# yangt1013/SPEINet

Measured on AMD Instinct MI355X. Metric: deblurred 720p frames/sec, higher is better.
Workload: dtype f16 (correlation top2)

## Files before the change

include/speinet_hip.h:

```cpp
#ifndef SPEINET_HIP_H
#define SPEINET_HIP_H

#include <stdint.h>

#ifdef __cplusplus
extern "C" {
#endif

typedef void* spei_stream_t;

#define SPEI_ACT_NONE 0
#define SPEI_ACT_RELU 1
#define SPEI_ACT_GELU 2

#define SPEI_F32 0
#define SPEI_BF16 1
#define SPEI_F16 2

#define SPEI_CONV 0
#define SPEI_CONV_TRANSPOSED 1

int spei_version(void);
const char* spei_last_error(void);
const char* spei_arch(void);

int spei_any_nonzero(const float* x, int64_t n, int32_t* flag, spei_stream_t stream);

int spei_rl_prior(const float* img, float* out, float* scratch, int C, int H, int W, int iters, float lam,
                  spei_stream_t stream);

int spei_conv5_in(const float* img_chw, const float* w, const float* bias, float* out_hwc, int H, int W,
                  int Cout, spei_stream_t stream);

int spei_conv5_out(const float* in_hwc, int ldi, const float* w, const float* bias, float* out_chw, int H,
                   int W, int Cin, spei_stream_t stream);

int spei_igemm_f32(const float* a0, int lda0, int k0, const float* a1, int lda1, int k1, const float* w,
                   const float* bias, float* out, int ldo, const float* residual, int ldr,
                   const float* rowscale, int Hin, int Win, int Hout, int Wout, int N, int ksize, int stride,
                   int pad, int mode, int act, spei_stream_t stream);

int spei_igemm_f32_batched(const float* a0, int lda0, int k0, const float* a1, int lda1, int k1, const float* w,
                           const float* bias, float* out, int ldo, const float* residual, int ldr,
                           const float* rowscale, int Hin, int Win, int Hout, int Wout, int N, int ksize, int stride,
                           int pad, int mode, int act, int batch, spei_stream_t stream);

int spei_conv_slab16(int fmt, const void* a0, int lda0, int k0, const void* a1, int lda1, int k1, int a_fmt,
                     const void* wfrag_hi, const void* wfrag_lo, const float* bias, void* out, int ldo, int out_fmt,
                     const float* residual, int ldr, const float* rowscale, int Hin, int Win, int Hout, int Wout,
                     int N, int ksize, int stride, int pad, int act, int ln_input, spei_stream_t stream);

int spei_conv_slab16_batched(int fmt, const void* a0, int k0, int a_fmt, const void* wfrag, const void* wfrag_lo, const float* bias,
                             void* out, int out_fmt, const float* residual, int batch, int Hin, int Win, int Hout, int Wout, int N,
                             int ksize, int stride, int pad, int act, spei_stream_t stream);

int spei_conv32_ws16(int fmt, const void* a, int a_fmt, const void* wfrag, const float* bias, void* out, int out_fmt, int batch,
                     int H, int W, int act, spei_stream_t stream);

int spei_conv64_ws16(int fmt, const void* a, int a_fmt, const void* wfrag, const float* bias, void* out, int out_fmt, int batch,
                     int H, int W, int act, spei_stream_t stream);

int spei_mlp_fused16(int fmt, const float* x, float* out, const void* w1_frag, const float* b1, const void* w2_frag,
                     const float* b2, int64_t M, spei_stream_t stream);

int spei_convt2_slab16(int fmt, const void* a0, int lda0, int k0, int a_fmt, const void* wfrag00, const void* wfrag01,
                       const void* wfrag10, const void* wfrag11, const float* bias, void* out, int ldo, int out_fmt,
                       int Hin, int Win, int N, int act, spei_stream_t stream);

int spei_convt2_slab16x3(const float* a0, int lda0, int k0, const void* const* whi4, const void* const* wlo4, const float* bias,
                         float* out, int ldo, int Hin, int Win, int N, int act, spei_stream_t stream);

int spei_conv3x3_256_pipe16(int fmt, const float* x, const void* w_frag, const float* bias, const float* residual, float* out,
                            int batch, int H, int W, spei_stream_t stream);

int spei_conv5_out_slab16(int fmt, const void* in, int ldi, int in_fmt, const void* wfrag, const float* bias32, float* out_chw,
                          int H, int W, spei_stream_t stream);

int spei_attn_fused16(int fmt, const float* x, float* out, const void* yhat, const void* wq_frag, const float* bq,
                      const void* wkv_frag, const float* bkv, const void* wproj_frag, const float* bproj,
                      const float* relbias, int H, int W, int shift, spei_stream_t stream);

int spei_attn_win4_16(int fmt, const float* x, float* out, const void* yhat, const void* wq_frag, const float* bq,
                      const void* wkv_frag, const float* bkv, const void* wproj_frag, const float* bproj,
                      const float* relbias, int batch, int H, int W, int shift, spei_stream_t stream);

int64_t spei_frame_metrics_ws_doubles(int H, int W, int border);
int spei_frame_metrics(const unsigned char* out_hwc, const unsigned char* gt_hwc, int H, int W, int border, double* ws, double* result,
                       spei_stream_t stream);

int64_t spei_gate_ws_floats(int H, int W, int C);
int spei_resblock_gates(const void* x1, int x1_fmt, int H, int W, int C, const float* se_w1, const float* se_b1,
                        const float* se_w2, const float* se_b2, const float* cw_w, const float* cw_bn,
                        const float* hc_w, const float* hc_bn, float* s, float* g1, float* g2, float* ws,
                        spei_stream_t stream);
int spei_resblock_apply(const float* x, const void* x1, int x1_fmt, const float* s, const float* g1, const float* g2,
                        const float* extra, float* out, int ldo, int H, int W, int C, spei_stream_t stream);

int spei_resblock_gates_batched(const void* x1, int x1_fmt, int batch, int H, int W, int C, const float* se_w1, const float* se_b1,
                                const float* se_w2, const float* se_b2, const float* cw_w, const float* cw_bn, const float* hc_w,
                                const float* hc_bn, float* s, float* g1, float* g2, float* ws, spei_stream_t stream);
int spei_resblock_apply_batched(const float* x, const void* x1, int x1_fmt, const float* s, const float* g1, const float* g2, float* out,
                                int batch, int H, int W, int C, spei_stream_t stream);

int spei_layernorm256(const float* x, void* y, int out_fmt, const float* gamma, const float* beta, int64_t M,
                      spei_stream_t stream);

int spei_window_attention(const void* q, const void* kv, int io_fmt, const float* relbias, void* out, int H, int W,
                          int shift, spei_stream_t stream);
int spei_window_attention_batched(const void* q, const void* kv, int io_fmt, const float* relbias, void* out, int H, int W,
                                  int shift, int batch, spei_stream_t stream);

int spei_patch_invnorm(const float* f, int ldf, float* inv, int H, int W, int C, spei_stream_t stream);

int64_t spei_corr_ws_floats(int64_t n_lr);
int spei_corr_argmax(const float* lr, int ldl, const float* ref, int ldr, const float* inv_lr,
                     const float* inv_ref, int Hl, int Wl, int Hr, int Wr, int C, float* S, int32_t* arg,
                     float* ws, spei_stream_t stream);

int spei_split16(int fmt, const float* x, int ld, void* hi, void* lo, int64_t M, int C, spei_stream_t stream);
int spei_corr_argmax_bf16(const void* lr_hi, const void* lr_lo, const void* ref_hi, const void* ref_lo,
                          const float* inv_lr, const float* inv_ref, int Hl, int Wl, int Hr, int Wr, int C, float* S,
                          int32_t* arg, float* ws, spei_stream_t stream);

int spei_corr_slab16(int fmt, const void* lr_hi, const void* lr_lo, const void* ref_hi, const void* ref_lo,
                     const float* inv_lr, const float* inv_ref, int Hl, int Wl, int Hr, int Wr, int C, float* S,
                     int32_t* arg, float* ws, spei_stream_t stream);

int spei_corr_slab_top2_16(int fmt, const void* lr16, const void* ref16, const float* inv_lr, const float* inv_ref,
                           int Hl, int Wl, int Hr, int Wr, int C, float* S, int32_t* arg, float* S2, int32_t* arg2,
                           float* ws, spei_stream_t stream);
int64_t spei_corr_diag_ws_floats(int Hl, int Wl, int Hr, int Wr);
int spei_corr_diag_top2_16(int fmt, const void* lr16, const void* ref16, const float* inv_ref, int Hl, int Wl, int Hr, int Wr,
                           int C, float* S, int32_t* arg, float* S2, int32_t* arg2, float* ws, spei_stream_t stream);
int spei_corr_rescore(const float* lr, int ldl, const float* ref, int ldr, const float* inv_lr, const float* inv_ref,
                      int Hl, int Wl, int Hr, int Wr, int C, float* S, int32_t* arg, const float* S2, const int32_t* arg2,
                      spei_stream_t stream);

int spei_gather_fold(const float* ref, int ldr, const int32_t* arg, float* out, int ldo, int H3, int W3,
                     int Hr3, int Wr3, int C, int s, spei_stream_t stream);

int spei_rot90(const float* in, int ldi, float* out, int H, int W, int C, spei_stream_t stream);

int spei_upsample_bicubic(const float* in, int ldi, float* out, int ldo, int H, int W, int C, int s, int act,
                          spei_stream_t stream);

int spei_add(const float* a, const float* b, float* out, int64_t n, spei_stream_t stream);


int64_t spei_wgrad_ws_floats(int Hout, int Wout, int N, int K, int ksize);
int spei_conv_wgrad_f32(const float* x, int ldx, const float* dy, int ldy, float* dw, float* dbias, float* ws, int Hin, int Win,
                        int Hout, int Wout, int N, int K, int ksize, int stride, int pad, spei_stream_t stream);

int spei_conv_wgrad_f32_batched(const float* x, int ldx, const float* dy, int ldy, float* dw, float* dbias, float* ws, int Hin, int Win,
                                int Hout, int Wout, int N, int K, int ksize, int stride, int pad, int batch, spei_stream_t stream);

int spei_pack_split16(const float* w, int N, int K, int ksize, int mode, void* frag_hi, void* frag_lo, spei_stream_t stream);

int spei_conv_wgrad_bf16x3_batched(const float* x, int ldx, const float* dy, int ldy, float* dw, float* dbias, float* ws, int Hin, int Win,
                                   int Hout, int Wout, int N, int K, int ksize, int stride, int pad, int batch, spei_stream_t stream);

int spei_conv_wgrad_bf16_batched(const float* x, int ldx, const float* dy, int ldy, float* dw, float* dbias, float* ws, int Hin, int Win,
                                 int Hout, int Wout, int N, int K, int ksize, int stride, int pad, int batch, spei_stream_t stream);

int spei_conv_s2_adjoint_slab16(const float* dy, int k0, const void* const* wfrag4, float* out, int N, int Hin, int Win, int ksize,
                                int batch, spei_stream_t stream);

int spei_relu_bwd(const float* y, const float* dy, float* dz, int64_t n, spei_stream_t stream);

int64_t spei_plane_ws_floats(int H, int W, int C);
int spei_plane_stats(const float* a, const float* b, int prod, int H, int W, int C, float* rowmax, int* rowarg, float* rowmean,
                     float* colmax, int* colarg, float* colmean, float* mean, float* ws, spei_stream_t stream);

int spei_plane_stats_batched(const float* a, const float* b, int prod, int H, int W, int C, float* rowmax, int* rowarg, float* rowmean,
                             float* colmax, int* colarg, float* colmean, float* mean, float* ws, int batch, spei_stream_t stream);

int spei_resblock_apply_bwd(const float* dout, const float* s, const float* g1, const float* g2, const int* rowarg, const int* colarg,
                            const float* d_rowmax, const float* d_rowmean, const float* d_colmax, const float* d_colmean,
                            const float* d_mean, float* dx1, int H, int W, int C, spei_stream_t stream);
int spei_resblock_apply_bwd_batched(const float* dout, const float* s, const float* g1, const float* g2, const int* rowarg,
                                    const int* colarg, const float* d_rowmax, const float* d_rowmean, const float* d_colmax,
                                    const float* d_colmean, const float* d_mean, float* dx1, int batch, int H, int W, int C,
                                    spei_stream_t stream);

int64_t spei_gate_train_saved_floats(int N, int groups, int H, int W, int C);
int64_t spei_gate_train_ws_floats(int N, int groups, int H, int W, int C);
int spei_gate_train_nparams(int C);
int spei_gate_maps_fwd(const float* rowmax, const float* rowmean, const float* colmax, const float* colmean, const float* mean,
                       const float* const* prm, float* const* run, int N, int groups, int H, int W, int C, int bn_train,
                       int update_running, float* s, float* g1, float* g2, float* saved, float* ws, spei_stream_t stream);
int spei_gate_maps_bwd(const float* rowmax, const float* rowmean, const float* colmax, const float* colmean, const float* mean,
                       const float* const* prm, float* const* run, int N, int groups, int H, int W, int C, int bn_train,
                       const float* s, const float* saved, const float* ds, const float* dg1, const float* dg2, float* d_rowmax,
                       float* d_rowmean, float* d_colmax, float* d_colmean, float* d_mean, float* dprm, float* ws,
                       spei_stream_t stream);


int64_t spei_ln_bwd_blocks(int64_t M);
int spei_layernorm256_bwd(const float* x, const float* gamma, const float* dy, float* dx, float* part, int64_t M, spei_stream_t stream);

int spei_gelu_fwd(const float* pre, float* out, int64_t n, spei_stream_t stream);
int spei_gelu_bwd(const float* pre, const float* dy, float* dpre, int64_t n, spei_stream_t stream);

int spei_window_attention_bwd(const float* q, const float* kv, const float* relbias, const float* dout, float* dq, float* dkv,
                              float* dbias_part, int H, int W, int shift, int batch, spei_stream_t stream);

int spei_window_attention16_train(const float* q, const float* kv, const float* relbias, float* out, int H, int W, int shift, int batch,
                                  spei_stream_t stream);
int spei_window_attention16_bwd(const float* q, const float* kv, const float* relbias, const float* dout, float* dq, float* dkv,
                                float* dbias_part, int H, int W, int shift, int batch, spei_stream_t stream);

int spei_scale_rows(const float* x, const float* rowscale, float* out, int64_t M, int N, spei_stream_t stream);


int spei_corr_s_bwd_lr(const float* lr, const float* ref, const float* inv_lr, const float* inv_ref, const float* S, const int32_t* arg,
                       const float* dS, float* dlr, int H, int W, int Hr, int Wr, int C, spei_stream_t stream);

int spei_search_bwd_ref(const float* ref, const float* dT, const float* lr, const float* inv_lr, const float* inv_ref, const float* S,
                        const float* dS, const int32_t* order, const int32_t* start, float* dref, int H3, int W3, int Hr3, int Wr3,
                        int C, int s, spei_stream_t stream);

int spei_upsample_bicubic_bwd(const float* dy, float* dx, int H, int W, int C, int s, spei_stream_t stream);

int spei_rowdot(const float* a, const float* b, float* out, int64_t M, int N, spei_stream_t stream);

int spei_det_gray(const float* rgb, float* gray, int N, int H, int W, spei_stream_t stream);
int64_t spei_det_ws_floats(int N, int H, int W, int k);
int spei_det_features(const float* gray, float* out, float* ws, int N, int H, int W, int k, spei_stream_t stream);


int spei_frames_u8_in(const unsigned char* src, int64_t frame_stride, float* dst, float* gray, int N, int H, int W, spei_stream_t stream);

int spei_frame_u8_out(const float* src, unsigned char* dst, int* nonfinite, int H, int W, int Hp, int Wp, spei_stream_t stream);

int spei_frame_pair_stats(const unsigned char* src, int64_t frame_stride, const unsigned char* prev, int N, int H, int W, int* hist,
                          int64_t* sad, spei_stream_t stream);

int spei_frames_u16_in(const uint16_t* src, int64_t frame_stride, float* dst, float* gray, int N, int H, int W, int depth,
                       spei_stream_t stream);
int spei_frame_u16_out(const float* src, uint16_t* dst, int* nonfinite, int H, int W, int Hp, int Wp, int depth, spei_stream_t stream);
int spei_frame_pair_stats_u16(const uint16_t* src, int64_t frame_stride, const uint16_t* prev, int N, int H, int W, int depth, int* hist,
                              int64_t* sad, spei_stream_t stream);


#define SPEI_YUV_420_CENTER 0
#define SPEI_YUV_420_LEFT 1
#define SPEI_YUV_444 2
#define SPEI_YUV_BT601 0
#define SPEI_YUV_BT709 1
#define SPEI_YUV_FULL 0
#define SPEI_YUV_LIMITED 1

int spei_yuv_to_rgb_u8(const unsigned char* src, int64_t frame_stride, unsigned char* dst, int N, int H, int W, int layout, int matrix,
                       int range, spei_stream_t stream);
int spei_rgb_u8_to_yuv(const unsigned char* src, unsigned char* dst, int H, int W, int layout, int matrix, int range,
                       spei_stream_t stream);

int spei_yuv_to_rgb_u16(const uint16_t* src, int64_t frame_stride, uint16_t* dst, int N, int H, int W, int layout, int matrix, int range,
                        int depth, spei_stream_t stream);
int spei_rgb_u16_to_yuv(const uint16_t* src, uint16_t* dst, int H, int W, int layout, int matrix, int range, int depth,
                        spei_stream_t stream);


#define SPEI_CROP_HFLIP 1
#define SPEI_CROP_VFLIP 2
#define SPEI_CROP_ROT90 4
#define SPEI_CROP_ZERO 8
typedef struct {
    uint64_t src;
    int32_t pitch;
    int32_t y0, x0;
    int32_t flags;
    int32_t H, W;
} spei_crop_record;

int spei_train_batch_u8(const spei_crop_record* table, const spei_crop_record* table_host, int n_in, int n_gt, float* input, float* gt,
                        int P, float rgb_range, spei_stream_t stream);

typedef struct {
    uint64_t src;
    int64_t frame_stride;
    int32_t pitch;
    int32_t y0, x0;
    int32_t flags;
    int32_t H, W;
    int32_t length;
    int32_t avail;
} spei_run_record;

int spei_train_batch_runs_u8(const spei_run_record* table, const spei_run_record* table_host, int n_in, int n_gt, float* input, float* gt,
                             int P, float rgb_range, spei_stream_t stream);

#define SPEI_PSNR_WS_DOUBLES 256
int spei_psnr_f32(const float* a, const float* b, int H, int W, int shave, float rgb_range, double* ws, double* result,
                  spei_stream_t stream);


int spei_window_mean_u8(const unsigned char* src, int64_t frame_stride, int T, const int* runs, const int* runs_host, int M,
                        unsigned char* blur, unsigned char* gt, float* gray, int H, int W, spei_stream_t stream);


int spei_window_mean_light_u8(const unsigned char* src, int64_t frame_stride, int T, const int* runs, const int* runs_host, int M,
                              const uint32_t* tables, const uint32_t* tables_host, unsigned char* blur, unsigned char* gt, float* gray,
                              int H, int W, spei_stream_t stream);

int spei_train_batch_runs_light_u8(const spei_run_record* table, const spei_run_record* table_host, int n_in, int n_gt,
                                   const uint32_t* tables, const uint32_t* tables_host, float* input, float* gt, int P, float rgb_range,
                                   spei_stream_t stream);

#ifdef __cplusplus
}
#endif
#endif
```

speinet_amd/csrc/resblock.hip:

```cpp
#include "common.h"

namespace {

constexpr int GATE_TR16 = 16;
constexpr int GATE_TR32 = 8;
__host__ __device__ inline int gate_tr(bool lp) { return lp ? GATE_TR16 : GATE_TR32; }
__host__ __device__ inline int gate_tc(int C) { return 256 / (C / 8); }

struct GateWs {
    float* rowpmax;
    float* rowpsum;
    float* colpmax;
    float* colpsum;
    float* tilesum;
    int ntx, nty;
};
__host__ __device__ inline GateWs carve(float* ws, int H, int W, int C, bool lp) {
    GateWs g;
    g.ntx = (W + gate_tc(C) - 1) / gate_tc(C);
    g.nty = (H + gate_tr(lp) - 1) / gate_tr(lp);
    g.rowpmax = ws;
    g.rowpsum = g.rowpmax + (size_t)g.ntx * H * C;
    g.colpmax = g.rowpsum + (size_t)g.ntx * H * C;
    g.colpsum = g.colpmax + (size_t)g.nty * W * C;
    g.tilesum = g.colpsum + (size_t)g.nty * W * C;
    return g;
}

template <typename T>
__device__ __forceinline__ f32x4 ld4(const T* p) {
    if constexpr (sizeof(T) == 4) {
        return *reinterpret_cast<const f32x4*>(p);
    } else {
        const typename lpv<T>::x4 h = *reinterpret_cast<const typename lpv<T>::x4*>(p);
        return f32x4{(float)h[0], (float)h[1], (float)h[2], (float)h[3]};
    }
}

__device__ __forceinline__ f32x4 max4(f32x4 a, f32x4 b) {
    return f32x4{fmaxf(a[0], b[0]), fmaxf(a[1], b[1]), fmaxf(a[2], b[2]), fmaxf(a[3], b[3])};
}

template <int C, typename TX>
__global__ __launch_bounds__(256) void gate_stats_kernel(const TX* __restrict__ x1, int H, int W, float* ws, int64_t wsf) {
    constexpr bool LP = sizeof(TX) == 2;
    x1 += (size_t)blockIdx.y * H * W * C;
    const GateWs g = carve(ws + (size_t)blockIdx.y * wsf, H, W, C, LP);
    constexpr int OCT = C / 8;
    constexpr int TC = 256 / OCT;
    constexpr int TR = LP ? GATE_TR16 : GATE_TR32;
    constexpr int EB = LP ? 16 : 32;
    constexpr int ROWB = TC * OCT * EB + 4 * EB;
    constexpr int ITEMS = TR * OCT;
    constexpr int PARTS = 256 / ITEMS;
    constexpr int SEG = TC / PARTS;
    extern __shared__ __attribute__((aligned(16))) unsigned char tile[];
    float* rsum = reinterpret_cast<float*>(tile + TR * ROWB);
    const int tid = threadIdx.x;
    const int oct = tid % OCT, col = tid / OCT;
    const int tx = blockIdx.x % g.ntx, ty = blockIdx.x / g.ntx;
    const int x = tx * TC + col, y0 = ty * TR;

    u32x4 v[TR][LP ? 1 : 2];
#pragma unroll
    for (int r = 0; r < TR; ++r) {
        const bool ok = x < W && y0 + r < H;
        const TX* src = x1 + ((size_t)min(y0 + r, H - 1) * W + min(x, W - 1)) * C + oct * 8;
#pragma unroll
        for (int hlf = 0; hlf < (LP ? 1 : 2); ++hlf) {
            v[r][hlf] = *reinterpret_cast<const u32x4*>(reinterpret_cast<const unsigned char*>(src) + 16 * hlf);
            if (!ok) v[r][hlf] = u32x4{0u, 0u, 0u, 0u};
        }
    }
    auto unpack = [](const u32x4* q, float* f) __attribute__((always_inline)) {
        if constexpr (LP) {
            const typename lpv<TX>::x8 h = *reinterpret_cast<const typename lpv<TX>::x8*>(q);
#pragma unroll
            for (int e = 0; e < 8; ++e) f[e] = (float)h[e];
        } else {
#pragma unroll
            for (int e = 0; e < 8; ++e) f[e] = __uint_as_float(q[e >> 2][e & 3]);
        }
    };
    float cmax[8], csum[8];
#pragma unroll
    for (int e = 0; e < 8; ++e) { cmax[e] = -INFINITY; csum[e] = 0.f; }
#pragma unroll
    for (int r = 0; r < TR; ++r) {
        float f[8];
        unpack(v[r], f);
        if (y0 + r < H) {
#pragma unroll
            for (int e = 0; e < 8; ++e) { cmax[e] = fmaxf(cmax[e], f[e]); csum[e] += f[e]; }
        }
#pragma unroll
        for (int hlf = 0; hlf < (LP ? 1 : 2); ++hlf)
            *reinterpret_cast<u32x4*>(tile + r * ROWB + (col * OCT + oct) * EB + 16 * hlf) = v[r][hlf];
    }
    if (x < W) {
        float* pm = g.colpmax + ((size_t)ty * W + x) * C + oct * 8;
        float* ps = g.colpsum + ((size_t)ty * W + x) * C + oct * 8;
        *reinterpret_cast<f32x4*>(pm) = f32x4{cmax[0], cmax[1], cmax[2], cmax[3]};
        *reinterpret_cast<f32x4*>(pm + 4) = f32x4{cmax[4], cmax[5], cmax[6], cmax[7]};
        *reinterpret_cast<f32x4*>(ps) = f32x4{csum[0], csum[1], csum[2], csum[3]};
        *reinterpret_cast<f32x4*>(ps + 4) = f32x4{csum[4], csum[5], csum[6], csum[7]};
    }
    __syncthreads();

    {
        const int part = tid % PARTS, item = tid / PARTS;
        const int ro = item % OCT, rr = item / OCT;
        float rmax[8], rs[8];
#pragma unroll
        for (int e = 0; e < 8; ++e) { rmax[e] = -INFINITY; rs[e] = 0.f; }
        const int ncol = min(TC, W - tx * TC);
#pragma unroll 4
        for (int j = 0; j < SEG; ++j) {
            const int c2 = j * PARTS + part;
            u32x4 q[LP ? 1 : 2];
#pragma unroll
            for (int hlf = 0; hlf < (LP ? 1 : 2); ++hlf) q[hlf] = *reinterpret_cast<const u32x4*>(tile + rr * ROWB + (c2 * OCT + ro) * EB + 16 * hlf);
            float f[8];
            unpack(q, f);
            if (c2 < ncol) {
#pragma unroll
                for (int e = 0; e < 8; ++e) { rmax[e] = fmaxf(rmax[e], f[e]); rs[e] += f[e]; }
            }
        }
#pragma unroll
        for (int e = 0; e < 8; ++e) {
            if constexpr (PARTS >= 2) { rmax[e] = fmaxf(rmax[e], dpp_quad<0xB1>(rmax[e])); rs[e] += dpp_quad<0xB1>(rs[e]); }
            if constexpr (PARTS >= 4) { rmax[e] = fmaxf(rmax[e], dpp_quad<0x4E>(rmax[e])); rs[e] += dpp_quad<0x4E>(rs[e]); }
            if constexpr (PARTS >= 8) { rmax[e] = fmaxf(rmax[e], dpp_quad<0x141>(rmax[e])); rs[e] += dpp_quad<0x141>(rs[e]); }
        }
        const int y = y0 + rr;
        if (part == 0) {
#pragma unroll
            for (int e = 0; e < 8; ++e) rsum[rr * C + ro * 8 + e] = (y < H) ? rs[e] : 0.f;
            if (y < H) {
                float* pm = g.rowpmax + ((size_t)tx * H + y) * C + ro * 8;
                float* ps = g.rowpsum + ((size_t)tx * H + y) * C + ro * 8;
                *reinterpret_cast<f32x4*>(pm) = f32x4{rmax[0], rmax[1], rmax[2], rmax[3]};
                *reinterpret_cast<f32x4*>(pm + 4) = f32x4{rmax[4], rmax[5], rmax[6], rmax[7]};
                *reinterpret_cast<f32x4*>(ps) = f32x4{rs[0], rs[1], rs[2], rs[3]};
                *reinterpret_cast<f32x4*>(ps + 4) = f32x4{rs[4], rs[5], rs[6], rs[7]};
            }
        }
    }
    __syncthreads();
    if (tid < C) {
        float t = 0.f;
#pragma unroll
        for (int r = 0; r < TR; ++r) t += rsum[r * C + tid];
        g.tilesum[(size_t)blockIdx.x * C + tid] = t;
    }
}

template <int C, typename TX>
void launch_gate_stats(const TX* x1, int H, int W, const GateWs& g, float* ws, int64_t wsf, int batch, hipStream_t st) {
    constexpr bool LP = sizeof(TX) == 2;
    constexpr int OCT = C / 8, TC = 256 / OCT, TR = LP ? GATE_TR16 : GATE_TR32, EB = LP ? 16 : 32;
    const size_t lds = (size_t)TR * (TC * OCT * EB + 4 * EB) + (size_t)TR * C * sizeof(float);
    ensure_dyn_lds<&gate_stats_kernel<C, TX>>(lds);
    hipLaunchKernelGGL((gate_stats_kernel<C, TX>), dim3(g.ntx * g.nty, batch), dim3(256), lds, st, x1, H, W, ws, wsf);
}

__device__ __forceinline__ void reduce_partials(const float* __restrict__ pmax, const float* __restrict__ psum, int nt, int64_t stride,
                                                int l0, int cnt, int L, int C, float, float denom, float* zmax, float* zmean) {
    float mx[4], sm[4];
    int64_t off[4];
    bool ok[4];
#pragma unroll
    for (int j = 0; j < 4; ++j) {
        const int it = threadIdx.x + 256 * j;
        const int line = l0 + it / C;
        ok[j] = it < cnt * C && line >= 0 && line < L;
        off[j] = ok[j] ? (int64_t)line * C + it % C : 0;
        mx[j] = -INFINITY;
        sm[j] = 0.f;
    }
    int k = 0;
    for (; k + 4 <= nt; k += 4) {
        float a[4][4], b[4][4];
#pragma unroll
        for (int u = 0; u < 4; ++u)
#pragma unroll
            for (int j = 0; j < 4; ++j) {
                a[u][j] = pmax[(size_t)(k + u) * stride + off[j]];
                b[u][j] = psum[(size_t)(k + u) * stride + off[j]];
            }
#pragma unroll
        for (int u = 0; u < 4; ++u)
#pragma unroll
            for (int j = 0; j < 4; ++j) { mx[j] = fmaxf(mx[j], a[u][j]); sm[j] += b[u][j]; }
    }
    for (; k < nt; ++k) {
#pragma unroll
        for (int j = 0; j < 4; ++j) {
            const float a = pmax[(size_t)k * stride + off[j]], b = psum[(size_t)k * stride + off[j]];
            mx[j] = fmaxf(mx[j], a);
            sm[j] += b;
        }
    }
#pragma unroll
    for (int j = 0; j < 4; ++j) {
        const int it = threadIdx.x + 256 * j;
        if (it < cnt * C) {
            zmax[it] = ok[j] ? mx[j] : -INFINITY;
            zmean[it] = ok[j] ? sm[j] / denom : 0.f;
        }
    }
}

__global__ __launch_bounds__(256) void gate_maps_kernel(int H, int W, int C, float* ws, int64_t wsf, int lp, const float* __restrict__ cw_w,
                                                        const float* __restrict__ cw_bn, const float* __restrict__ hc_w,
                                                        const float* __restrict__ hc_bn, float* __restrict__ g1,
                                                        float* __restrict__ g2, const float* __restrict__ w1,
                                                        const float* __restrict__ b1, const float* __restrict__ w2,
                                                        const float* __restrict__ b2, float* __restrict__ s) {
    const GateWs g = carve(ws + (size_t)blockIdx.y * wsf, H, W, C, lp != 0);
    g1 += (size_t)blockIdx.y * H * C;
    g2 += (size_t)blockIdx.y * W * C;
    s += (size_t)blockIdx.y * C;
    __shared__ float wk[98];
    __shared__ float zmax[1024], zmean[1024];
    const int64_t n1 = (int64_t)H * C;
    const int nb1 = (int)((n1 + 255) / 256);
    const int nb2 = (int)(((int64_t)W * C + 255) / 256);
    if ((int)blockIdx.x == nb1 + nb2) {
        __shared__ f32x4 part[256];
        __shared__ float mean[128], hid[32];
        const int ntiles = g.ntx * g.nty, cq = C / 4, parts = 256 / cq;
        const int q = threadIdx.x % cq, pt = threadIdx.x / cq;
        const f32x4* ts = reinterpret_cast<const f32x4*>(g.tilesum) + q;
        f32x4 acc[8];
#pragma unroll
        for (int u = 0; u < 8; ++u) acc[u] = f32x4{0.f, 0.f, 0.f, 0.f};
        int t = pt;
        for (; t + 7 * parts < ntiles; t += 8 * parts) {
#pragma unroll
            for (int u = 0; u < 8; ++u) acc[u] += ts[(size_t)(t + u * parts) * cq];
        }
        for (; t < ntiles; t += parts) acc[0] += ts[(size_t)t * cq];
        part[threadIdx.x] = ((acc[0] + acc[1]) + (acc[2] + acc[3])) + ((acc[4] + acc[5]) + (acc[6] + acc[7]));
        __syncthreads();
        if ((int)threadIdx.x < C) {
            const int c = threadIdx.x;
            float a = 0.f;
            for (int k = 0; k < parts; ++k) a += part[k * cq + (c >> 2)][c & 3];
            mean[c] = a / ((float)H * (float)W);
        }
        __syncthreads();
        const int mid = C / 4;
        if ((int)threadIdx.x < mid) {
            float a = b1[threadIdx.x];
            for (int k = 0; k < C; ++k) a = fmaf(w1[threadIdx.x * C + k], mean[k], a);
            hid[threadIdx.x] = fmaxf(a, 0.f);
        }
        __syncthreads();
        if ((int)threadIdx.x < C) {
            float a = b2[threadIdx.x];
            for (int k = 0; k < mid; ++k) a = fmaf(w2[threadIdx.x * mid + k], hid[k], a);
            s[threadIdx.x] = 1.0f / (1.0f + expf(-a));
        }
        return;
    }
    if ((int)blockIdx.x < nb1) {
        if (threadIdx.x < 98) wk[threadIdx.x] = cw_w[threadIdx.x];
        const int64_t i0 = (int64_t)blockIdx.x * 256;
        const int y0 = (int)(i0 / C) - 3, rows = 256 / C + 6;
        reduce_partials(g.rowpmax, g.rowpsum, g.ntx, n1, y0, rows, H, C, 1.0f, (float)W, zmax, zmean);
        __syncthreads();
        const int64_t i = i0 + threadIdx.x;
        if (i >= n1) return;
        const int c = (int)(i % C), y = (int)(i / C);
        float acc = 0.f;
#pragma unroll
        for (int ch = 0; ch < 2; ++ch) {
            const float* z = ch == 0 ? zmax : zmean;
            for (int dy = 0; dy < 7; ++dy) {
                const int yy = y + dy - 3;
                if (yy < 0 || yy >= H) continue;
                for (int dc = 0; dc < 7; ++dc) {
                    const int cc = c + dc - 3;
                    if (cc < 0 || cc >= C) continue;
                    acc = fmaf(wk[ch * 49 + dy * 7 + dc], z[(yy - y0) * C + cc], acc);
                }
            }
        }
        g1[i] = fmaf(acc, cw_bn[0], cw_bn[1]);
    } else {
        if (threadIdx.x < 50) wk[threadIdx.x] = hc_w[threadIdx.x];
        const int64_t n2 = (int64_t)W * C;
        const int64_t i0 = (int64_t)(blockIdx.x - nb1) * 256;
        const int x0 = (int)(i0 / C) - 2, cols = 256 / C + 4;
        reduce_partials(g.colpmax, g.colpsum, g.nty, n2, x0, cols, W, C, 1.0f, (float)H, zmax, zmean);
        __syncthreads();
        const int64_t i = i0 + threadIdx.x;
        if (i >= n2) return;
        const int c = (int)(i % C), x = (int)(i / C);
        float acc = 0.f;
#pragma unroll
        for (int ch = 0; ch < 2; ++ch) {
            const float* z = ch == 0 ? zmax : zmean;
            for (int dc = 0; dc < 5; ++dc) {
                const int cc = c + dc - 2;
                if (cc < 0 || cc >= C) continue;
                for (int dx = 0; dx < 5; ++dx) {
                    const int xx = x + dx - 2;
                    if (xx < 0 || xx >= W) continue;
                    acc = fmaf(wk[ch * 25 + dc * 5 + dx], z[(xx - x0) * C + cc], acc);
                }
            }
        }
        g2[i] = fmaf(acc, hc_bn[0], hc_bn[1]);
    }
}

template <typename T>
__global__ __launch_bounds__(256) void resblock_apply_kernel(const float* __restrict__ x, const T* __restrict__ x1,
                                                             const float* __restrict__ s, const float* __restrict__ g1,
                                                             const float* __restrict__ g2, const float* __restrict__ extra,
                                                             float* __restrict__ out, int ldo, int H, int W, int C) {
    const int cg = C / 4;
    const int64_t total = (int64_t)H * W * cg;
    {
        const size_t b = blockIdx.y;
        x += b * H * W * C; x1 += b * H * W * C; out += b * H * W * ldo;
        s += b * C; g1 += b * H * C; g2 += b * W * C;
    }
    for (int64_t i = (int64_t)blockIdx.x * 256 + threadIdx.x; i < total; i += (int64_t)gridDim.x * 256) {
        const int c = (int)(i % cg) * 4;
        const int64_t pix = i / cg;
        const int xx = (int)(pix % W), yy = (int)(pix / W);
        const float4 a = *reinterpret_cast<const float4*>(x + pix * C + c);
        const f32x4 bv = ld4<T>(x1 + pix * C + c);
        const float4 b = make_float4(bv[0], bv[1], bv[2], bv[3]);
        const float4 sv = *reinterpret_cast<const float4*>(s + c);
        const float4 u = *reinterpret_cast<const float4*>(g1 + (size_t)yy * C + c);
        const float4 v = *reinterpret_cast<const float4*>(g2 + (size_t)xx * C + c);
        float4 o;
        o.x = (b.x * sv.x + (b.x * u.x + b.x * v.x)) + a.x;
        o.y = (b.y * sv.y + (b.y * u.y + b.y * v.y)) + a.y;
        o.z = (b.z * sv.z + (b.z * u.z + b.z * v.z)) + a.z;
        o.w = (b.w * sv.w + (b.w * u.w + b.w * v.w)) + a.w;
        if (extra) {
            const float4 e = *reinterpret_cast<const float4*>(extra + pix * C + c);
            o.x += e.x; o.y += e.y; o.z += e.z; o.w += e.w;
        }
        *reinterpret_cast<float4*>(out + pix * ldo + c) = o;
    }
}

}

extern "C" int64_t spei_gate_ws_floats(int H, int W, int C) {
    if (C != 32 && C != 64 && C != 128) return 0;
    const int64_t ntx = (W + gate_tc(C) - 1) / gate_tc(C), nty = (H + GATE_TR32 - 1) / GATE_TR32;
    return 2 * ntx * H * C + 2 * nty * W * C + ntx * nty * C;
}

static int resblock_gates_run(const void* x1, int x1_fmt, int batch, int H, int W, int C, const float* se_w1, const float* se_b1,
                              const float* se_w2, const float* se_b2, const float* cw_w, const float* cw_bn,
                              const float* hc_w, const float* hc_bn, float* s, float* g1, float* g2, float* ws,
                              spei_stream_t stream) {
    SPEI_REQUIRE(batch >= 1 && batch <= 65535, "spei_resblock_gates_batched: batch=%d", batch);
    SPEI_REQUIRE(x1 && se_w1 && se_b1 && se_w2 && se_b2 && cw_w && cw_bn && hc_w && hc_bn && s && g1 && g2 && ws,
                 "spei_resblock_gates: null pointer");
    SPEI_REQUIRE(C == 32 || C == 64 || C == 128, "spei_resblock_gates: C=%d (32/64/128 built)", C);
    SPEI_REQUIRE(H > 0 && W > 0, "spei_resblock_gates: empty map");
    SPEI_REQUIRE(((uintptr_t)x1 | (uintptr_t)ws) % 16 == 0, "spei_resblock_gates: 16-byte alignment required");
    hipStream_t st = (hipStream_t)stream;
    SPEI_REQUIRE(x1_fmt == SPEI_F32 || x1_fmt == SPEI_BF16 || x1_fmt == SPEI_F16, "spei_resblock_gates: x1_fmt=%d", x1_fmt);
    GateWs g = carve(ws, H, W, C, x1_fmt != SPEI_F32);
    const int64_t wsf = spei_gate_ws_floats(H, W, C);
    if (x1_fmt == SPEI_BF16) {
        const __bf16* xp = (const __bf16*)x1;
        if (C == 32) launch_gate_stats<32>(xp, H, W, g, ws, wsf, batch, st);
        else if (C == 64) launch_gate_stats<64>(xp, H, W, g, ws, wsf, batch, st);
        else launch_gate_stats<128>(xp, H, W, g, ws, wsf, batch, st);
    } else if (x1_fmt == SPEI_F16) {
        const _Float16* xp = (const _Float16*)x1;
        if (C == 32) launch_gate_stats<32>(xp, H, W, g, ws, wsf, batch, st);
        else if (C == 64) launch_gate_stats<64>(xp, H, W, g, ws, wsf, batch, st);
        else launch_gate_stats<128>(xp, H, W, g, ws, wsf, batch, st);
    } else {
        const float* xp = (const float*)x1;
        if (C == 32) launch_gate_stats<32>(xp, H, W, g, ws, wsf, batch, st);
        else if (C == 64) launch_gate_stats<64>(xp, H, W, g, ws, wsf, batch, st);
        else launch_gate_stats<128>(xp, H, W, g, ws, wsf, batch, st);
    }
    hipLaunchKernelGGL(gate_maps_kernel, dim3(cdiv((int64_t)H * C, 256) + cdiv((int64_t)W * C, 256) + 1, batch), dim3(256), 0, st, H, W, C, ws, wsf,
                       (int)(x1_fmt != SPEI_F32), cw_w, cw_bn, hc_w, hc_bn, g1, g2, se_w1, se_b1, se_w2, se_b2, s);
    SPEI_CHECK_LAUNCH("spei_resblock_gates");
    return 0;
}

extern "C" int spei_resblock_gates(const void* x1, int x1_fmt, int H, int W, int C, const float* se_w1, const float* se_b1,
                                   const float* se_w2, const float* se_b2, const float* cw_w, const float* cw_bn,
                                   const float* hc_w, const float* hc_bn, float* s, float* g1, float* g2, float* ws,
                                   spei_stream_t stream) {
    return resblock_gates_run(x1, x1_fmt, 1, H, W, C, se_w1, se_b1, se_w2, se_b2, cw_w, cw_bn, hc_w, hc_bn, s, g1, g2, ws, stream);
}

extern "C" int spei_resblock_gates_batched(const void* x1, int x1_fmt, int batch, int H, int W, int C, const float* se_w1, const float* se_b1,
                                           const float* se_w2, const float* se_b2, const float* cw_w, const float* cw_bn,
                                           const float* hc_w, const float* hc_bn, float* s, float* g1, float* g2, float* ws,
                                           spei_stream_t stream) {
    return resblock_gates_run(x1, x1_fmt, batch, H, W, C, se_w1, se_b1, se_w2, se_b2, cw_w, cw_bn, hc_w, hc_bn, s, g1, g2, ws, stream);
}

static int resblock_apply_run(const float* x, const void* x1, int x1_fmt, const float* s, const float* g1, const float* g2,
                              const float* extra, float* out, int ldo, int batch, int H, int W, int C, spei_stream_t stream) {
    SPEI_REQUIRE(x && x1 && s && g1 && g2 && out, "spei_resblock_apply: null pointer");
    SPEI_REQUIRE(batch >= 1 && batch <= 65535 && (batch == 1 || (!extra && ldo == C)), "spei_resblock_apply_batched: dense maps, no `extra`");
    SPEI_REQUIRE(C % 4 == 0 && ldo % 4 == 0 && ldo >= C && H > 0 && W > 0, "spei_resblock_apply: bad shape");
    const int64_t total = (int64_t)H * W * (C / 4);
    const int blocks = (int)((total + 255) / 256 < 8192 ? (total + 255) / 256 : 8192);
    const dim3 grid(blocks, batch);
    SPEI_REQUIRE(x1_fmt == SPEI_F32 || x1_fmt == SPEI_BF16 || x1_fmt == SPEI_F16, "spei_resblock_apply: x1_fmt=%d", x1_fmt);
    if (x1_fmt == SPEI_BF16) hipLaunchKernelGGL(resblock_apply_kernel<__bf16>, grid, dim3(256), 0, (hipStream_t)stream, x, (const __bf16*)x1, s, g1, g2, extra, out, ldo, H, W, C);
    else if (x1_fmt == SPEI_F16) hipLaunchKernelGGL(resblock_apply_kernel<_Float16>, grid, dim3(256), 0, (hipStream_t)stream, x, (const _Float16*)x1, s, g1, g2, extra, out, ldo, H, W, C);
    else hipLaunchKernelGGL(resblock_apply_kernel<float>, grid, dim3(256), 0, (hipStream_t)stream, x, (const float*)x1, s, g1, g2, extra, out, ldo, H, W, C);
    SPEI_CHECK_LAUNCH("spei_resblock_apply");
    return 0;
}

extern "C" int spei_resblock_apply(const float* x, const void* x1, int x1_fmt, const float* s, const float* g1, const float* g2,
                                   const float* extra, float* out, int ldo, int H, int W, int C, spei_stream_t stream) {
    return resblock_apply_run(x, x1, x1_fmt, s, g1, g2, extra, out, ldo, 1, H, W, C, stream);
}

extern "C" int spei_resblock_apply_batched(const float* x, const void* x1, int x1_fmt, const float* s, const float* g1, const float* g2,
                                           float* out, int batch, int H, int W, int C, spei_stream_t stream) {
    return resblock_apply_run(x, x1, x1_fmt, s, g1, g2, nullptr, out, C, batch, H, W, C, stream);
}
```

speinet_amd/csrc/stencil.hip:

```cpp
#include <stdarg.h>
#include <string.h>
#include "common.h"

static thread_local char g_err[512] = "";
void spei_set_error(const char* fmt, ...) {
    va_list ap;
    va_start(ap, fmt);
    vsnprintf(g_err, sizeof(g_err), fmt, ap);
    va_end(ap);
}
extern "C" const char* spei_last_error(void) { return g_err; }
extern "C" int spei_version(void) { return 100; }
extern "C" const char* spei_arch(void) { return "gfx950"; }

__global__ void any_nonzero_kernel(const float* __restrict__ x, int64_t n, int32_t* flag) {
    int64_t i = (int64_t)blockIdx.x * blockDim.x + threadIdx.x;
    const int64_t step = (int64_t)gridDim.x * blockDim.x;
    bool nz = false;
    for (; i < n; i += step) nz |= (x[i] != 0.0f);
    if (__any(nz) && (threadIdx.x & 63) == 0) atomicOr(flag, 1);
}
extern "C" int spei_any_nonzero(const float* x, int64_t n, int32_t* flag, spei_stream_t stream) {
    SPEI_REQUIRE(x && flag && n > 0, "spei_any_nonzero: bad arguments");
    hipStream_t s = (hipStream_t)stream;
    (void)hipMemsetAsync(flag, 0, sizeof(int32_t), s);
    const int blocks = (int)((n + 256 * 16 - 1) / (256 * 16));
    hipLaunchKernelGGL(any_nonzero_kernel, dim3(blocks < 2048 ? blocks : 2048), dim3(256), 0, s, x, n, flag);
    SPEI_CHECK_LAUNCH("spei_any_nonzero");
    return 0;
}

constexpr int RL_T = 32;
__global__ __launch_bounds__(256) void rl_iter_kernel(const float* __restrict__ img, const float* __restrict__ d,
                                                      float* __restrict__ out, int H, int W, float lam) {
    __shared__ float t[RL_T + 4][RL_T + 4 + 1];
    const size_t plane = (size_t)blockIdx.z * H * W;
    const int x0 = blockIdx.x * RL_T, y0 = blockIdx.y * RL_T;
    for (int i = threadIdx.x; i < (RL_T + 4) * (RL_T + 4); i += 256) {
        const int ly = i / (RL_T + 4), lx = i - ly * (RL_T + 4);
        const int gy = y0 + ly - 2, gx = x0 + lx - 2;
        t[ly][lx] = (gy >= 0 && gy < H && gx >= 0 && gx < W) ? d[plane + (size_t)gy * W + gx] : 0.0f;
    }
    __syncthreads();
    const int lx = threadIdx.x & 31;
    for (int ly = threadIdx.x >> 5; ly < RL_T; ly += 8) {
        const int gy = y0 + ly, gx = x0 + lx;
        if (gy >= H || gx >= W) continue;
        float b = 0.0f;
#pragma unroll
        for (int dy = 0; dy < 5; ++dy)
#pragma unroll
            for (int dx = 0; dx < 5; ++dx) b = fmaf(t[ly + dy][lx + dx], 0.04f, b);
        const float c0 = t[ly + 2][lx + 2];
        float lap = -t[ly + 1][lx + 2];
        lap -= t[ly + 2][lx + 1];
        lap = fmaf(4.0f, c0, lap);
        lap -= t[ly + 2][lx + 3];
        lap -= t[ly + 3][lx + 2];
        const float I = img[plane + (size_t)gy * W + gx];
        float c = I / b;
        if (c != c) c = 0.0f;
        if (c < 0.0f) c = 0.0f;
        out[plane + (size_t)gy * W + gx] = c * (c0 + lam * lap);
    }
}
extern "C" int spei_rl_prior(const float* img, float* out, float* scratch, int C, int H, int W, int iters, float lam,
                             spei_stream_t stream) {
    SPEI_REQUIRE(img && out && scratch && C > 0 && H > 0 && W > 0 && iters >= 1, "spei_rl_prior: bad arguments");
    SPEI_REQUIRE(out != img && scratch != img && out != scratch, "spei_rl_prior: buffers must be distinct");
    hipStream_t s = (hipStream_t)stream;
    dim3 grid(cdiv(W, RL_T), cdiv(H, RL_T), C);
    const float* src = img;
    for (int it = 0; it < iters; ++it) {
        float* dst = ((iters - 1 - it) % 2 == 0) ? out : scratch;
        hipLaunchKernelGGL(rl_iter_kernel, grid, dim3(256), 0, s, img, src, dst, H, W, lam);
        src = dst;
    }
    SPEI_CHECK_LAUNCH("spei_rl_prior");
    return 0;
}

constexpr int CI_TH = 8, CI_TW = 32, CI_P = CI_TW + 4 + 1;
__global__ __launch_bounds__(256) void conv5_in_kernel(const float* __restrict__ img, const float* __restrict__ w,
                                                       const float* __restrict__ bias, float* __restrict__ out,
                                                       int H, int W, int tiles_x, int ntiles) {
    __shared__ float tin[3 * (CI_TH + 4) * CI_P];
    const int tid = threadIdx.x, lane = tid & 63, wave = tid >> 6;
    const int fr = lane & 31, fk = lane >> 5;
    int koff[38];
    float bw[38];
#pragma unroll
    for (int kk = 0; kk < 38; ++kk) {
        const int k = 2 * kk + fk;
        const int t = k / 3, ci = k - 3 * t;
        const int dy = t / 5, dx = t - 5 * dy;
        koff[kk] = k < 75 ? (ci * (CI_TH + 4) + dy) * CI_P + dx : 0;
        bw[kk] = k < 75 ? w[(t * 32 + fr) * 3 + ci] : 0.0f;
    }
    const float bv = bias[fr];
    const float* a0 = tin + (wave * 2) * CI_P + fr;
    const int et = fr & 3, ecol = (fr >> 2) * 4;
    for (int tile = blockIdx.x; tile < ntiles; tile += gridDim.x) {
        const int ty = tile / tiles_x, tx = tile - ty * tiles_x;
        const int x0 = tx * CI_TW, y0 = ty * CI_TH;
        for (int i = tid; i < 3 * (CI_TH + 4) * (CI_TW + 4); i += 256) {
            const int c = i / ((CI_TH + 4) * (CI_TW + 4));
            const int r = i - c * (CI_TH + 4) * (CI_TW + 4);
            const int ly = r / (CI_TW + 4), lx = r - ly * (CI_TW + 4);
            const int gy = y0 + ly - 2, gx = x0 + lx - 2;
            tin[(c * (CI_TH + 4) + ly) * CI_P + lx] = (gy >= 0 && gy < H && gx >= 0 && gx < W) ? img[((size_t)c * H + gy) * W + gx] : 0.0f;
        }
        __syncthreads();
        float av[2][38];
#pragma unroll
        for (int kk = 0; kk < 38; ++kk) {
            av[0][kk] = a0[koff[kk]];
            av[1][kk] = a0[koff[kk] + CI_P];
        }
        __syncthreads();
        f32x16 acc[2];
#pragma unroll
        for (int i = 0; i < 2; ++i)
#pragma unroll
            for (int r = 0; r < 16; ++r) acc[i][r] = 0.f;
#pragma unroll
        for (int kk = 0; kk < 38; ++kk) {
            acc[0] = __builtin_amdgcn_mfma_f32_32x32x2f32(av[0][kk], bw[kk], acc[0], 0, 0, 0);
            acc[1] = __builtin_amdgcn_mfma_f32_32x32x2f32(av[1][kk], bw[kk], acc[1], 0, 0, 0);
        }
#pragma unroll
        for (int i = 0; i < 2; ++i) {
            const int gy = y0 + wave * 2 + i;
#pragma unroll
            for (int k = 0; k < 4; ++k) {
                float a[4];
#pragma unroll
                for (int e = 0; e < 4; ++e) a[e] = fmaxf(acc[i][4 * k + e] + bv, 0.f);
                quad_transpose4(a[0], a[1], a[2], a[3], et);
                const int gx = x0 + 8 * k + 4 * fk + et;
                if (gy < H && gx < W) *reinterpret_cast<f32x4*>(out + ((size_t)gy * W + gx) * 32 + ecol) = f32x4{a[0], a[1], a[2], a[3]};
            }
        }
    }
}
extern "C" int spei_conv5_in(const float* img_chw, const float* w, const float* bias, float* out_hwc, int H, int W,
                             int Cout, spei_stream_t stream) {
    SPEI_REQUIRE(img_chw && w && bias && out_hwc && H > 0 && W > 0, "spei_conv5_in: bad arguments");
    SPEI_REQUIRE(Cout == 32, "spei_conv5_in: Cout=%d (only n_feat=32 is built)", Cout);
    const int tiles_x = cdiv(W, CI_TW), ntiles = tiles_x * cdiv(H, CI_TH);
    hipLaunchKernelGGL(conv5_in_kernel, dim3(ntiles < 1024 ? ntiles : 1024), dim3(256), 0, (hipStream_t)stream,
                       img_chw, w, bias, out_hwc, H, W, tiles_x, ntiles);
    SPEI_CHECK_LAUNCH("spei_conv5_in");
    return 0;
}

constexpr int CO_TH = 8, CO_TW = 32, CO_P = 36;
__global__ __launch_bounds__(256) void conv5_out_kernel(const float* __restrict__ in, int ldi, const float* __restrict__ w,
                                                        const float* __restrict__ bias, float* __restrict__ out,
                                                        int H, int W) {
    extern __shared__ __attribute__((aligned(16))) float sm[];
    float* tin = sm;
    float* wl = sm + (CO_TH + 4) * (CO_TW + 4) * CO_P;
    const int x0 = blockIdx.x * CO_TW, y0 = blockIdx.y * CO_TH;
    for (int i = threadIdx.x; i < (CO_TH + 4) * (CO_TW + 4) * 8; i += 256) {
        const int pix = i >> 3, q = i & 7;
        const int ly = pix / (CO_TW + 4), lx = pix - ly * (CO_TW + 4);
        const int gy = y0 + ly - 2, gx = x0 + lx - 2;
        float4 v = make_float4(0.f, 0.f, 0.f, 0.f);
        if (gy >= 0 && gy < H && gx >= 0 && gx < W) v = *reinterpret_cast<const float4*>(in + ((size_t)gy * W + gx) * ldi + q * 4);
        *reinterpret_cast<float4*>(tin + pix * CO_P + q * 4) = v;
    }
    for (int i = threadIdx.x; i < 25 * 3 * 32; i += 256) {
        const int t = i / 96, r = i - t * 96, co = r / 32, ci = r - co * 32;
        wl[(co * 25 + t) * 32 + ci] = w[i];
    }
    __syncthreads();
    const int lx = threadIdx.x & 31, ly = threadIdx.x >> 5;
    const int gy = y0 + ly, gx = x0 + lx;
    float a0 = bias[0], a1 = bias[1], a2 = bias[2];
    for (int t = 0; t < 25; ++t) {
        const int dy = t / 5, dx = t - dy * 5;
        const float4* pin = reinterpret_cast<const float4*>(tin + ((ly + dy) * (CO_TW + 4) + lx + dx) * CO_P);
        const float4* w0 = reinterpret_cast<const float4*>(wl + (0 * 25 + t) * 32);
        const float4* w1 = reinterpret_cast<const float4*>(wl + (1 * 25 + t) * 32);
        const float4* w2 = reinterpret_cast<const float4*>(wl + (2 * 25 + t) * 32);
#pragma unroll
        for (int q = 0; q < 8; ++q) {
            const float4 v = pin[q];
            const float4 u0 = w0[q], u1 = w1[q], u2 = w2[q];
            a0 = fmaf(v.x, u0.x, a0); a0 = fmaf(v.y, u0.y, a0); a0 = fmaf(v.z, u0.z, a0); a0 = fmaf(v.w, u0.w, a0);
            a1 = fmaf(v.x, u1.x, a1); a1 = fmaf(v.y, u1.y, a1); a1 = fmaf(v.z, u1.z, a1); a1 = fmaf(v.w, u1.w, a1);
            a2 = fmaf(v.x, u2.x, a2); a2 = fmaf(v.y, u2.y, a2); a2 = fmaf(v.z, u2.z, a2); a2 = fmaf(v.w, u2.w, a2);
        }
    }
    if (gy < H && gx < W) {
        const size_t o = (size_t)gy * W + gx, hw = (size_t)H * W;
        out[o] = a0; out[hw + o] = a1; out[2 * hw + o] = a2;
    }
}
extern "C" int spei_conv5_out(const float* in_hwc, int ldi, const float* w, const float* bias, float* out_chw, int H,
                              int W, int Cin, spei_stream_t stream) {
    SPEI_REQUIRE(in_hwc && w && bias && out_chw && H > 0 && W > 0, "spei_conv5_out: bad arguments");
    SPEI_REQUIRE(Cin == 32 && ldi % 4 == 0 && ldi >= 32, "spei_conv5_out: Cin=%d ldi=%d (only n_feat=32 is built)", Cin, ldi);
    const size_t lds = ((size_t)(CO_TH + 4) * (CO_TW + 4) * CO_P + 3 * 25 * 32) * sizeof(float);
    ensure_dyn_lds<&conv5_out_kernel>(lds);
    hipLaunchKernelGGL(conv5_out_kernel, dim3(cdiv(W, CO_TW), cdiv(H, CO_TH)), dim3(256), lds, (hipStream_t)stream,
                       in_hwc, ldi, w, bias, out_chw, H, W);
    SPEI_CHECK_LAUNCH("spei_conv5_out");
    return 0;
}

__device__ __forceinline__ void cubic_coeffs(float t, float c[4]) {
    const float A = -0.75f;
    float x = t + 1.0f;
    c[0] = ((A * x - 5.0f * A) * x + 8.0f * A) * x - 4.0f * A;
    x = t;
    c[1] = ((A + 2.0f) * x - (A + 3.0f)) * x * x + 1.0f;
    x = 1.0f - t;
    c[2] = ((A + 2.0f) * x - (A + 3.0f)) * x * x + 1.0f;
    x = 2.0f - t;
    c[3] = ((A * x - 5.0f * A) * x + 8.0f * A) * x - 4.0f * A;
}
template <int VEC>
__global__ __launch_bounds__(256) void bicubic_kernel(const float* __restrict__ in, int ldi, float* __restrict__ out, int ldo,
                                                      int H, int W, int C, int s, int relu) {
    const int cg = C / VEC;
    const int64_t total = (int64_t)H * s * W * s * cg;
    const float scale = 1.0f / (float)s;
    for (int64_t i = (int64_t)blockIdx.x * 256 + threadIdx.x; i < total; i += (int64_t)gridDim.x * 256) {
        const int c = (int)(i % cg) * VEC;
        const int64_t pix = i / cg;
        const int ox = (int)(pix % (W * s)), oy = (int)(pix / (W * s));
        const float ry = scale * ((float)oy + 0.5f) - 0.5f, rx = scale * ((float)ox + 0.5f) - 0.5f;
        const float fy = floorf(ry), fx = floorf(rx);
        float cy[4], cx[4];
        cubic_coeffs(ry - fy, cy);
        cubic_coeffs(rx - fx, cx);
        const int iy = (int)fy, ix = (int)fx;
        float acc[VEC];
#pragma unroll
        for (int a = 0; a < 4; ++a) {
            const int yy = min(max(iy - 1 + a, 0), H - 1);
            float row[VEC];
#pragma unroll
            for (int b = 0; b < 4; ++b) {
                const int xx = min(max(ix - 1 + b, 0), W - 1);
                const float* p = in + ((size_t)yy * W + xx) * ldi + c;
                if (VEC == 4) {
                    const float4 v = *reinterpret_cast<const float4*>(p);
                    const float vv[4] = {v.x, v.y, v.z, v.w};
#pragma unroll
                    for (int e = 0; e < VEC; ++e) row[e] = (b == 0) ? vv[e] * cx[0] : fmaf(vv[e], cx[b], row[e]);
                } else {
                    row[0] = (b == 0) ? p[0] * cx[0] : fmaf(p[0], cx[b], row[0]);
                }
            }
#pragma unroll
            for (int e = 0; e < VEC; ++e) acc[e] = (a == 0) ? row[e] * cy[0] : fmaf(row[e], cy[a], acc[e]);
        }
        if (relu) {
#pragma unroll
            for (int e = 0; e < VEC; ++e) acc[e] = fmaxf(acc[e], 0.f);
        }
        float* o = out + ((size_t)oy * (W * s) + ox) * ldo + c;
        if (VEC == 4) *reinterpret_cast<float4*>(o) = make_float4(acc[0], acc[1], acc[2], acc[3]);
        else o[0] = acc[0];
    }
}
__global__ __launch_bounds__(256) void bicubic2x_kernel(const float* __restrict__ in, int ldi, float* __restrict__ out, int ldo,
                                                        int H, int W, int C, int relu) {
    const int cg = C / 4;
    const int64_t total = (int64_t)H * W * cg;
    float ce[4], co[4];
    cubic_coeffs(0.75f, ce);
    cubic_coeffs(0.25f, co);
    for (int64_t i = (int64_t)blockIdx.x * 256 + threadIdx.x; i < total; i += (int64_t)gridDim.x * 256) {
        const int c = (int)(i % cg) * 4;
        const int64_t pix = i / cg;
        const int x = (int)(pix % W), y = (int)(pix / W);
        int xs[5];
#pragma unroll
        for (int b = 0; b < 5; ++b) xs[b] = min(max(x - 2 + b, 0), W - 1);
        f32x4 he[5], ho[5];
#pragma unroll
        for (int a = 0; a < 5; ++a) {
            const int yy = min(max(y - 2 + a, 0), H - 1);
            const float* rowp = in + (size_t)yy * W * ldi + c;
            f32x4 v[5];
#pragma unroll
            for (int b = 0; b < 5; ++b) v[b] = *reinterpret_cast<const f32x4*>(rowp + (size_t)xs[b] * ldi);
#pragma unroll
            for (int e = 0; e < 4; ++e) {
                float re = v[0][e] * ce[0], ro = v[1][e] * co[0];
#pragma unroll
                for (int b = 1; b < 4; ++b) { re = fmaf(v[b][e], ce[b], re); ro = fmaf(v[b + 1][e], co[b], ro); }
                he[a][e] = re;
                ho[a][e] = ro;
            }
        }
#pragma unroll
        for (int py = 0; py < 2; ++py)
#pragma unroll
            for (int px = 0; px < 2; ++px) {
                const f32x4* h = px ? ho : he;
                const float* cy = py ? co : ce;
                f32x4 acc;
#pragma unroll
                for (int e = 0; e < 4; ++e) {
                    float r = h[py][e] * cy[0];
#pragma unroll
                    for (int a = 1; a < 4; ++a) r = fmaf(h[py + a][e], cy[a], r);
                    acc[e] = relu ? fmaxf(r, 0.f) : r;
                }
                *reinterpret_cast<f32x4*>(out + ((size_t)(2 * y + py) * (2 * W) + 2 * x + px) * ldo + c) = acc;
            }
    }
}

extern "C" int spei_upsample_bicubic(const float* in, int ldi, float* out, int ldo, int H, int W, int C, int s, int act,
                                     spei_stream_t stream) {
    SPEI_REQUIRE(in && out && H > 0 && W > 0 && C > 0 && (s == 2 || s == 4), "spei_upsample_bicubic: bad arguments");
    SPEI_REQUIRE(act == SPEI_ACT_NONE || act == SPEI_ACT_RELU, "spei_upsample_bicubic: act=%d", act);
    SPEI_REQUIRE(ldi >= C && ldo >= C, "spei_upsample_bicubic: bad row strides");
    const bool v4 = (C % 4 == 0) && (ldi % 4 == 0) && (ldo % 4 == 0);
    if (v4 && s == 2 && ((uintptr_t)in | (uintptr_t)out) % 16 == 0) {
        const int64_t tot2 = (int64_t)H * W * (C / 4);
        const int blocks2 = (int)((tot2 + 255) / 256 < 8192 ? (tot2 + 255) / 256 : 8192);
        hipLaunchKernelGGL(bicubic2x_kernel, dim3(blocks2), dim3(256), 0, (hipStream_t)stream, in, ldi, out, ldo, H, W, C, act == SPEI_ACT_RELU);
        SPEI_CHECK_LAUNCH("spei_upsample_bicubic");
        return 0;
    }
    const int64_t total = (int64_t)H * s * W * s * (v4 ? C / 4 : C);
    const int blocks = (int)((total + 255) / 256 < 8192 ? (total + 255) / 256 : 8192);
    if (v4) hipLaunchKernelGGL(bicubic_kernel<4>, dim3(blocks), dim3(256), 0, (hipStream_t)stream, in, ldi, out, ldo, H, W, C, s, act == SPEI_ACT_RELU);
    else    hipLaunchKernelGGL(bicubic_kernel<1>, dim3(blocks), dim3(256), 0, (hipStream_t)stream, in, ldi, out, ldo, H, W, C, s, act == SPEI_ACT_RELU);
    SPEI_CHECK_LAUNCH("spei_upsample_bicubic");
    return 0;
}

__global__ __launch_bounds__(256) void rot90_kernel(const float* __restrict__ in, int ldi, float* __restrict__ out, int H, int W, int C) {
    const int cg = C / 4;
    const int64_t total = (int64_t)H * W * cg;
    for (int64_t i = (int64_t)blockIdx.x * 256 + threadIdx.x; i < total; i += (int64_t)gridDim.x * 256) {
        const int c = (int)(i % cg) * 4;
        const int64_t pix = i / cg;
        const int b = (int)(pix % H), a = (int)(pix / H);
        *reinterpret_cast<float4*>(out + ((size_t)a * H + b) * C + c) =
            *reinterpret_cast<const float4*>(in + ((size_t)b * W + (W - 1 - a)) * ldi + c);
    }
}
extern "C" int spei_rot90(const float* in, int ldi, float* out, int H, int W, int C, spei_stream_t stream) {
    SPEI_REQUIRE(in && out && H > 0 && W > 0 && C % 4 == 0 && ldi % 4 == 0, "spei_rot90: bad arguments");
    const int64_t total = (int64_t)H * W * (C / 4);
    const int blocks = (int)((total + 255) / 256 < 8192 ? (total + 255) / 256 : 8192);
    hipLaunchKernelGGL(rot90_kernel, dim3(blocks), dim3(256), 0, (hipStream_t)stream, in, ldi, out, H, W, C);
    SPEI_CHECK_LAUNCH("spei_rot90");
    return 0;
}

__global__ __launch_bounds__(256) void add_kernel(const float* __restrict__ a, const float* __restrict__ b, float* __restrict__ o, int64_t n4, int64_t n) {
    for (int64_t i = (int64_t)blockIdx.x * 256 + threadIdx.x; i < n4; i += (int64_t)gridDim.x * 256) {
        const float4 x = reinterpret_cast<const float4*>(a)[i], y = reinterpret_cast<const float4*>(b)[i];
        reinterpret_cast<float4*>(o)[i] = make_float4(x.x + y.x, x.y + y.y, x.z + y.z, x.w + y.w);
    }
    if (blockIdx.x == 0) for (int64_t i = n4 * 4 + threadIdx.x; i < n; i += 256) o[i] = a[i] + b[i];
}
extern "C" int spei_add(const float* a, const float* b, float* out, int64_t n, spei_stream_t stream) {
    SPEI_REQUIRE(a && b && out && n > 0, "spei_add: bad arguments");
    SPEI_REQUIRE(((uintptr_t)a | (uintptr_t)b | (uintptr_t)out) % 16 == 0, "spei_add: 16-byte alignment required");
    const int64_t n4 = n / 4;
    const int blocks = (int)((n4 + 255) / 256 < 4096 ? (n4 + 255) / 256 : 4096);
    hipLaunchKernelGGL(add_kernel, dim3(blocks > 0 ? blocks : 1), dim3(256), 0, (hipStream_t)stream, a, b, out, n4, n);
    SPEI_CHECK_LAUNCH("spei_add");
    return 0;
}
```

speinet_amd/csrc/swin.hip:

```cpp
#include "common.h"

namespace {

template <typename TO>
__global__ __launch_bounds__(256) void layernorm256_kernel(const float* __restrict__ x, TO* __restrict__ y,
                                                           const float* __restrict__ gamma, const float* __restrict__ beta,
                                                           int64_t M) {
    const int lane = threadIdx.x & 63;
    const int64_t wave = (int64_t)blockIdx.x * 4 + (threadIdx.x >> 6);
    const int64_t nwaves = (int64_t)gridDim.x * 4;
    float4 g = make_float4(1.f, 1.f, 1.f, 1.f), b = make_float4(0.f, 0.f, 0.f, 0.f);
    if (gamma) g = reinterpret_cast<const float4*>(gamma)[lane];
    if (beta) b = reinterpret_cast<const float4*>(beta)[lane];
    for (int64_t m = wave; m < M; m += nwaves) {
        const float4 v = reinterpret_cast<const float4*>(x + m * 256)[lane];
        const float mean = wave_sum((v.x + v.y) + (v.z + v.w)) * (1.0f / 256.0f);
        const float dx = v.x - mean, dy = v.y - mean, dz = v.z - mean, dw = v.w - mean;
        const float var = wave_sum((dx * dx + dy * dy) + (dz * dz + dw * dw)) * (1.0f / 256.0f);
        const float rstd = 1.0f / sqrtf(var + 1e-5f);
        float4 o;
        o.x = dx * rstd * g.x + b.x;
        o.y = dy * rstd * g.y + b.y;
        o.z = dz * rstd * g.z + b.z;
        o.w = dw * rstd * g.w + b.w;
        if (sizeof(TO) == 4) {
            reinterpret_cast<float4*>(y + m * 256)[lane] = o;
        } else {
            typename lpv<TO>::x4 h;
            h[0] = (TO)o.x; h[1] = (TO)o.y; h[2] = (TO)o.z; h[3] = (TO)o.w;
            reinterpret_cast<typename lpv<TO>::x4*>(y + m * 256)[lane] = h;
        }
    }
}

constexpr int WS = 5, NT = 25, HD = 32, LDT = HD + 1;

__device__ __forceinline__ int mask_region(int v, int n, int shift) {
    return v < n - WS ? 0 : (v < n - shift ? 1 : 2);
}

template <typename T>
__device__ __forceinline__ float4 load4(const T* p) {
    if constexpr (sizeof(T) == 4) {
        return *reinterpret_cast<const float4*>(p);
    } else {
        const typename lpv<T>::x4 h = *reinterpret_cast<const typename lpv<T>::x4*>(p);
        return make_float4((float)h[0], (float)h[1], (float)h[2], (float)h[3]);
    }
}

template <typename T>
__global__ __launch_bounds__(256) void window_attention_kernel(const T* __restrict__ q, const T* __restrict__ kv,
                                                               const float* __restrict__ relbias, T* __restrict__ out,
                                                               int H, int W, int shift) {
    __shared__ float sQ[4][32][LDT], sK[4][32][LDT], sV[4][32][LDT];
    __shared__ int tok_pix[32], tok_reg[32];
    {
        const size_t z = (size_t)blockIdx.y * H * W;
        q += z * 256; kv += z * 512; out += z * 256;
    }
    const int wave = threadIdx.x >> 6, lane = threadIdx.x & 63;
    const int nwx = W / WS;
    const int win = blockIdx.x >> 1;
    const int wy = win / nwx, wx = win - wy * nwx;
    if (threadIdx.x < 32) {
        int pix = 0, reg = 0;
        if (threadIdx.x < NT) {
            const int ys = wy * WS + threadIdx.x / WS, xs = wx * WS + threadIdx.x % WS;
            int yo = ys + shift, xo = xs + shift;
            if (yo >= H) yo -= H;
            if (xo >= W) xo -= W;
            pix = yo * W + xo;
            reg = shift > 0 ? 3 * mask_region(ys, H, shift) + mask_region(xs, W, shift) : 0;
        }
        tok_pix[threadIdx.x] = pix;
        tok_reg[threadIdx.x] = reg;
    }
    __syncthreads();
    const int h = (blockIdx.x & 1) * 4 + wave;
    const int hl = wave;
    for (int i = lane; i < 32 * 8; i += 64) {
        const int r = i >> 3, c4 = (i & 7) * 4;
        float4 vq = make_float4(0.f, 0.f, 0.f, 0.f), vk = vq, vv = vq;
        if (r < NT) {
            const size_t p = (size_t)tok_pix[r];
            vq = load4<T>(q + p * 256 + h * HD + c4);
            vk = load4<T>(kv + p * 512 + h * HD + c4);
            vv = load4<T>(kv + p * 512 + 256 + h * HD + c4);
        }
        float* d = &sQ[hl][r][c4]; d[0] = vq.x; d[1] = vq.y; d[2] = vq.z; d[3] = vq.w;
        d = &sK[hl][r][c4];        d[0] = vk.x; d[1] = vk.y; d[2] = vk.z; d[3] = vk.w;
        d = &sV[hl][r][c4];        d[0] = vv.x; d[1] = vv.y; d[2] = vv.z; d[3] = vv.w;
    }
    __syncthreads();
    const int fr = lane & 31, fk = lane >> 5;
    f32x16 st;
#pragma unroll
    for (int r = 0; r < 16; ++r) st[r] = 0.f;
#pragma unroll
    for (int kk = 0; kk < HD; kk += 2)
        st = __builtin_amdgcn_mfma_f32_32x32x2f32(sK[hl][fr][kk + fk], sQ[hl][fr][kk + fk], st, 0, 0, 0);
    const int qi = fr < NT ? fr : 0;
    const int qreg = tok_reg[qi];
    float mx = -INFINITY;
#pragma unroll
    for (int r = 0; r < 16; ++r) {
        const int key = (r & 3) + 8 * (r >> 2) + 4 * fk;
        float v = -INFINITY;
        if (key < NT) {
            v = st[r] + relbias[(h * NT + qi) * NT + key];
            if (shift > 0 && tok_reg[key] != qreg) v += -100.0f;
        }
        st[r] = v;
        mx = fmaxf(mx, v);
    }
    mx = fmaxf(mx, __shfl_xor(mx, 32, 64));
    float sum = 0.f;
#pragma unroll
    for (int r = 0; r < 16; ++r) {
        const float e = expf(st[r] - mx);
        st[r] = e;
        sum += e;
    }
    sum += __shfl_xor(sum, 32, 64);
    const float inv = 1.0f / sum;
    f32x16 o;
#pragma unroll
    for (int r = 0; r < 16; ++r) o[r] = 0.f;
#pragma unroll
    for (int r = 0; r < 16; ++r) {
        const int key = (r & 3) + 8 * (r >> 2) + 4 * fk;
        o = __builtin_amdgcn_mfma_f32_32x32x2f32(st[r] * inv, sV[hl][key][fr], o, 0, 0, 0);
    }
#pragma unroll
    for (int r = 0; r < 16; ++r) {
        const int qq = (r & 3) + 8 * (r >> 2) + 4 * fk;
        if (qq < NT) out[(size_t)tok_pix[qq] * 256 + h * HD + fr] = (T)o[r];
    }
}

}

extern "C" int spei_layernorm256(const float* x, void* y, int out_fmt, const float* gamma, const float* beta, int64_t M,
                                 spei_stream_t stream) {
    SPEI_REQUIRE(x && y && M > 0, "spei_layernorm256: bad arguments");
    SPEI_REQUIRE(out_fmt == SPEI_F32 || out_fmt == SPEI_BF16 || out_fmt == SPEI_F16, "spei_layernorm256: out_fmt=%d", out_fmt);
    const int64_t blocks = (M + 3) / 4;
    const dim3 grid((unsigned)(blocks < 8192 ? blocks : 8192));
    if (out_fmt == SPEI_BF16) hipLaunchKernelGGL(layernorm256_kernel<__bf16>, grid, dim3(256), 0, (hipStream_t)stream, x, (__bf16*)y, gamma, beta, M);
    else if (out_fmt == SPEI_F16) hipLaunchKernelGGL(layernorm256_kernel<_Float16>, grid, dim3(256), 0, (hipStream_t)stream, x, (_Float16*)y, gamma, beta, M);
    else hipLaunchKernelGGL(layernorm256_kernel<float>, grid, dim3(256), 0, (hipStream_t)stream, x, (float*)y, gamma, beta, M);
    SPEI_CHECK_LAUNCH("spei_layernorm256");
    return 0;
}

static int window_attention_run(const void* q, const void* kv, int io_fmt, const float* relbias, void* out, int H, int W, int shift, int batch,
                                spei_stream_t stream) {
    SPEI_REQUIRE(q && kv && relbias && out, "spei_window_attention: null pointer");
    SPEI_REQUIRE(batch >= 1 && batch <= 65535, "spei_window_attention: batch=%d", batch);
    SPEI_REQUIRE(H > 0 && W > 0 && H % WS == 0 && W % WS == 0, "spei_window_attention: %dx%d is not a multiple of the 5x5 window", H, W);
    SPEI_REQUIRE(shift >= 0 && shift < WS, "spei_window_attention: shift=%d", shift);
    SPEI_REQUIRE(io_fmt == SPEI_F32 || io_fmt == SPEI_BF16 || io_fmt == SPEI_F16, "spei_window_attention: io_fmt=%d", io_fmt);
    const dim3 grid(2 * (H / WS) * (W / WS), batch);
    if (io_fmt == SPEI_BF16) hipLaunchKernelGGL(window_attention_kernel<__bf16>, grid, dim3(256), 0, (hipStream_t)stream, (const __bf16*)q, (const __bf16*)kv, relbias, (__bf16*)out, H, W, shift);
    else if (io_fmt == SPEI_F16) hipLaunchKernelGGL(window_attention_kernel<_Float16>, grid, dim3(256), 0, (hipStream_t)stream, (const _Float16*)q, (const _Float16*)kv, relbias, (_Float16*)out, H, W, shift);
    else hipLaunchKernelGGL(window_attention_kernel<float>, grid, dim3(256), 0, (hipStream_t)stream, (const float*)q, (const float*)kv, relbias, (float*)out, H, W, shift);
    SPEI_CHECK_LAUNCH("spei_window_attention");
    return 0;
}

extern "C" int spei_window_attention(const void* q, const void* kv, int io_fmt, const float* relbias, void* out, int H, int W,
                                     int shift, spei_stream_t stream) {
    return window_attention_run(q, kv, io_fmt, relbias, out, H, W, shift, 1, stream);
}

extern "C" int spei_window_attention_batched(const void* q, const void* kv, int io_fmt, const float* relbias, void* out, int H, int W,
                                             int shift, int batch, spei_stream_t stream) {
    return window_attention_run(q, kv, io_fmt, relbias, out, H, W, shift, batch, stream);
}
```

speinet_amd/engine.py:

```python
from __future__ import annotations

import contextlib
from functools import partial

import torch

from .ops import ACT_GELU, ACT_RELU, CONV_T, BMap, Ctx, FMap


def _resblocks(ctx: Ctx, f: FMap, blocks, extra=None, out=None) -> FMap:
    n = len(blocks)
    for i, pk in enumerate(blocks):
        last = i == n - 1
        f = ctx.resblock(f, pk, extra=extra if last else None, out=out if last else None)
    return f


def in_block(ctx: Ctx, frame: torch.Tensor, pk: dict) -> FMap:
    ctx = ctx.for_stage("enc")
    return _resblocks(ctx, ctx.conv5_in(frame, pk["head_w"], pk["head_b"]), pk["blocks"])


def enc_stage(ctx: Ctx, f: FMap, pk: dict, extra=None, out=None) -> FMap:
    ctx = ctx.for_stage("enc")
    n = pk["head_b"].numel()
    f = ctx.igemm(f, pk["head_w"], pk["head_b"], n, ksize=5, stride=2, act=ACT_RELU)
    return _resblocks(ctx, f, pk["blocks"], extra, out)


def enc(ctx: Ctx, frame: torch.Tensor, P: dict, extra=None, out=None) -> FMap:
    return enc_stage(ctx, enc_stage(ctx, in_block(ctx, frame, P["inBlock"]), P["encoder_first"]), P["encoder_second"], extra, out)


def enc_batched(ctx: Ctx, frames: list, P: dict):
    ctx = ctx.for_stage("enc")
    assert ctx.batched_available()
    b, (h, w) = len(frames), frames[0].shape[-2:]
    ib = P["inBlock"]
    lv1 = BMap.empty(b, h, w, ib["head_b"].numel(), frames[0].device)
    lib_in = lambda i: ctx.conv5_in(frames[i], ib["head_w"], ib["head_b"], out=lv1.map(i))
    for i in range(b):
        lib_in(i)
    for pk in ib["blocks"]:
        lv1 = ctx.resblock_batched(lv1, pk)
    levels = [lv1]
    f = lv1
    for name in ("encoder_first", "encoder_second"):
        st = P[name]
        f = ctx.igemm_batched(f, st["head_w"], st["head_b"], st["head_b"].numel(), 5, stride=2, act=ACT_RELU)
        for pk in st["blocks"]:
            f = ctx.resblock_batched(f, pk)
        levels.append(f)
    return levels


def dec_stage(ctx: Ctx, f: FMap, pk: dict) -> FMap:
    f = _resblocks(ctx, f, pk["blocks"])
    return ctx.for_stage("convt").igemm(f, pk["tail_w"], pk["tail_b"], pk["tail_b"].numel(), ksize=3, stride=2, mode=CONV_T, act=ACT_RELU)


class SwinX:

    def __init__(self, ctx: Ctx, f_mid: FMap, sw: dict):
        ctx = ctx.for_stage("swin")
        self.f_mid = f_mid
        self.x_first = ctx.igemm(f_mid, sw["conv_first_w"], sw["conv_first_b"], 256, ksize=3)
        self.xt0 = ctx.layernorm(self.x_first.t, sw["pe_g"], sw["pe_b"])


def swin(ctx: Ctx, sx: SwinX, feat: FMap, sw: dict, out: FMap) -> FMap:
    ctx = ctx.for_stage("swin")
    h, w = feat.H, feat.W
    m = h * w
    dev = feat.t.device
    y_first = ctx.igemm(feat, sw["conv_first_w"], sw["conv_first_b"], 256, ksize=3)
    yt = ctx.layernorm(y_first.t, sw["pe_g"], sw["pe_b"])
    idt = ctx.inter_dtype()
    yhat = ctx.layernorm(yt, out_dtype=idt)
    del y_first, yt
    r = sx.xt0.clone()
    bufs = [torch.empty(m, 256, device=dev), torch.empty(m, 256, device=dev)]
    xh = torch.empty(m, 256, device=dev, dtype=idt)
    q = torch.empty(m, 256, device=dev, dtype=idt)
    kv = torch.empty(m, 512, device=dev, dtype=idt)
    att = torch.empty(m, 256, device=dev, dtype=idt)
    hid = torch.empty(m, 512, device=dev, dtype=idt)
    for layer in sw["layers"]:
        cur = r
        for bi, bk in enumerate(layer["blocks"]):
            shift = 0 if bi % 2 == 0 else 2
            nxt = bufs[bi % 2]
            if ctx.attn_fused_available():
                ctx.attn_fused(cur, yhat, bk, h, w, shift, out=nxt)
            else:
                if ctx.ln_fused_available():
                    ctx.linear(cur, bk["wkv"], bk["bkv"], out=kv, ln_input=True)
                else:
                    ctx.layernorm(cur, out=xh)
                    ctx.linear(xh, bk["wkv"], bk["bkv"], out=kv)
                ctx.linear(yhat, bk["wq"], bk["bq"], out=q)
                ctx.window_attention(q, kv, bk["relbias"], h, w, shift, out=att)
                ctx.linear(att, bk["wproj"], bk["bproj"], residual=cur, out=nxt)
            if ctx.mlp_fused_available():
                ctx.mlp_fused(nxt, bk["w1"], bk["b1"], bk["w2"], bk["b2"], out=nxt)
            else:
                if ctx.ln_fused_available():
                    ctx.linear(nxt, bk["w1"], bk["b1"], act=ACT_GELU, out=hid, ln_input=True)
                else:
                    ctx.layernorm(nxt, out=xh)
                    ctx.linear(xh, bk["w1"], bk["b1"], act=ACT_GELU, out=hid)
                ctx.linear(hid, bk["w2"], bk["b2"], residual=nxt, out=nxt)
            cur = nxt
        rf = FMap(r, h, w, 256)
        ctx.igemm(FMap(cur, h, w, 256), layer["conv_w"], layer["conv_b"], 256, ksize=3, residual=rf, out=rf)
    xt = ctx.layernorm(r, sw["norm_g"], sw["norm_b"])
    res = ctx.igemm(FMap(xt, h, w, 256), sw["cab_w"], sw["cab_b"], 256, ksize=3, residual=sx.x_first)
    return ctx.igemm(res, sw["conv_last_w"], sw["conv_last_b"], 128, ksize=3, residual=sx.f_mid, out=out)


def swin_multi(ctx: Ctx, sx: SwinX, feats: BMap, sw: dict, outs: list) -> None:
    ctx = ctx.for_stage("swin")
    B, h, w = feats.B, feats.H, feats.W
    m = h * w
    dev = feats.t.device
    y_first = ctx.igemm_batched(feats, sw["conv_first_w"], sw["conv_first_b"], 256, 3)
    yt = ctx.layernorm(y_first.t, sw["pe_g"], sw["pe_b"])
    idt = ctx.inter_dtype()
    yhat = ctx.layernorm(yt, out_dtype=idt)
    del y_first, yt
    r = sx.xt0.repeat(B, 1)
    bufs = [torch.empty(B * m, 256, device=dev), torch.empty(B * m, 256, device=dev)]
    for layer in sw["layers"]:
        cur = r
        for bi, bk in enumerate(layer["blocks"]):
            shift = 0 if bi % 2 == 0 else 2
            nxt = bufs[bi % 2]
            ctx.attn_fused(cur, yhat, bk, h, w, shift, out=nxt)
            ctx.mlp_fused(nxt, bk["w1"], bk["b1"], bk["w2"], bk["b2"], out=nxt)
            cur = nxt
        rb = BMap(r, B, h, w, 256)
        ctx.igemm_batched(BMap(cur, B, h, w, 256), layer["conv_w"], layer["conv_b"], 256, 3, residual=rb, out=rb)
    xt = ctx.layernorm(r, sw["norm_g"], sw["norm_b"])
    x_first = BMap(sx.x_first.t.repeat(B, 1), B, h, w, 256)
    res = ctx.igemm_batched(BMap(xt, B, h, w, 256), sw["cab_w"], sw["cab_b"], 256, 3, residual=x_first)
    for b in range(B):
        ctx.igemm(res.map(b), sw["conv_last_w"], sw["conv_last_b"], 128, ksize=3, residual=sx.f_mid, out=outs[b])


def search_plan(ctx: Ctx, f_fusion: FMap, lv3: FMap):
    ctx = ctx.for_stage("search")
    return ctx.corr_plan(f_fusion, lv3, ctx.patch_invnorm(f_fusion), ctx.patch_invnorm(lv3))


def search_finish(ctx: Ctx, plan, f_fusion: FMap, lv1: FMap, lv2: FMap, lv3: FMap, return_arg=False):
    ctx = ctx.for_stage("search")
    s, arg = plan.s, plan.arg
    if ctx.capture is not None:
        ctx.capture.update(arg=arg, s=s)
    h3, w3 = f_fusion.H, f_fusion.W
    t3 = ctx.gather_fold(lv3, arg, h3, w3, lv3.H, lv3.W, 1)
    t2 = ctx.gather_fold(lv2, arg, h3, w3, lv3.H, lv3.W, 2)
    t1 = ctx.gather_fold(lv1, arg, h3, w3, lv3.H, lv3.W, 4)
    if return_arg:
        return s, t3, t2, t1, arg
    return s, t3, t2, t1


def search_transfer(ctx: Ctx, f_fusion: FMap, lv1: FMap, lv2: FMap, lv3: FMap, return_arg=False):
    plan = search_plan(ctx, f_fusion, lv3)
    plan.launch()
    return search_finish(ctx, plan, f_fusion, lv1, lv2, lv3, return_arg)


def self_plan(ctx: Ctx, f_fusion: FMap):
    ctx = ctx.for_stage("search")
    ref = ctx.rot90(f_fusion)
    return ctx.corr_plan(f_fusion, ref, ctx.patch_invnorm(f_fusion), ctx.patch_invnorm(ref))


def self_finish(ctx: Ctx, plan, f_fusion: FMap, P: dict):
    ctx = ctx.for_stage("search")
    s = plan.s
    if ctx.capture is not None:
        ctx.capture.update(s_self=s)
    p1, p2 = P["SelfTransfer.search1"], P["SelfTransfer.search2"]
    t2 = ctx.up_conv1x1_relu(f_fusion, p1["w"], p1["b"], 64)
    t1 = ctx.up_conv1x1_relu(t2, p2["w"], p2["b"], 32)
    return s, f_fusion, t2, t1


def self_transfer(ctx: Ctx, f_fusion: FMap, P: dict):
    plan = self_plan(ctx, f_fusion)
    plan.launch()
    return self_finish(ctx, plan, f_fusion, P)


def decode(ctx: Ctx, ff: FMap, s: torch.Tensor, t3: FMap, t2: FMap, t1: FMap, P: dict, out: torch.Tensor) -> torch.Tensor:
    ctx = ctx.for_stage("decode")
    g = ctx.for_stage("glue")
    g1 = ctx.for_stage("glue1")
    c = lambda name: (P[name]["w"], P[name]["b"])
    h3, w3 = ff.H, ff.W
    smap = FMap(s.view(h3 * w3, 1), h3, w3, 1)
    f_lv3 = g.igemm(ff, *c("conv_lv3"), 128, a1=t3, rowscale=s, residual=ff)
    dec2 = dec_stage(ctx.for_stage("dec2"), f_lv3, P["decoder_second"])
    s2 = ctx.upsample(smap, 2).t.view(-1)
    f_lv2 = g.igemm(dec2, *c("conv_lv2"), 64, a1=t2, rowscale=s2, residual=dec2)
    s1 = g.up_conv1x1_relu(f_lv3, *c("search1"), 64)
    sr2 = g.igemm(f_lv2, *c("search3"), 64, ksize=3, act=ACT_RELU)
    f_v3 = g.igemm(dec2, *c("search2"), 64, a1=s1, act=ACT_RELU, residual=dec2)
    f_lv2 = g.igemm(f_lv2, *c("search2"), 64, a1=sr2, act=ACT_RELU, residual=f_lv2)
    dec1 = dec_stage(ctx.for_stage("dec1"), f_lv2, P["decoder_first"])
    s4 = ctx.upsample(smap, 4).t.view(-1)
    f_lv1 = g1.igemm(dec1, *c("conv_lv1"), 32, a1=t1, rowscale=s4, residual=dec1)
    s13 = g.up_conv1x1_relu(f_v3, *c("search13"), 32)
    s23 = g1.igemm(ctx.upsample(f_lv2, 2), *c("search33"), 32, ksize=3, act=ACT_RELU)
    s33 = g1.igemm(f_lv1, *c("search43"), 32, ksize=3, act=ACT_RELU)
    acc = g1.igemm(s13, *c("search33"), 32, ksize=3, a1=s23, act=ACT_RELU, residual=f_lv1)
    g1.igemm(s13, *c("search33"), 32, ksize=3, a1=s33, act=ACT_RELU, residual=acc, out=acc)
    g1.igemm(s23, *c("search33"), 32, ksize=3, a1=s33, act=ACT_RELU, residual=acc, out=acc)
    ob = P["outBlock"]
    ctx = ctx.for_stage("out")
    f = _resblocks(ctx, acc, ob["blocks"])
    return ctx.for_stage("tail").conv5_out(f, ob["tail_w"], ob["tail_b"], out, ob.get("tail_w32"), ob.get("tail_b32"))


def model_streams(model, key: tuple, device, n: int) -> list:
    if key not in model._side_streams:
        model._side_streams[key] = [torch.cuda.Stream(device=device) for _ in range(n)]
    return model._side_streams[key]


def side_streams(model, device) -> list:
    n = max(1, int(model.streams)) - 1
    return model_streams(model, (torch.device(device).index, n), device, n)


def _lanes(ctx: Ctx, sides) -> list:
    return [torch.cuda.current_stream(ctx.device)] + list(sides or ())


@contextlib.contextmanager
def _side_lanes(lanes: list, fork: bool = True):
    main = lanes[0]
    for s_ in lanes[1:] if fork else ():
        s_.wait_stream(main)
    yield
    for s_ in lanes[1:]:
        main.wait_stream(s_)


def _swin_calls(ctx: Ctx, f_mid: FMap, ys: list, P: dict, cat: FMap, lanes: list) -> None:
    main = lanes[0]
    sx = SwinX(ctx, f_mid, P["swin"])
    ready = torch.cuda.Event()
    ready.record(main)
    for slot, y in enumerate(ys, start=1):
        lane = lanes[(slot - 1) % len(lanes)]
        with torch.cuda.stream(lane):
            feat = y() if callable(y) else y
            if lane is not main:
                lane.wait_event(ready)
            swin(ctx, sx, feat, P["swin"], out=cat.view(128 * slot, 128))


def forward_sample(ctx: Ctx, x: torch.Tensor, P: dict, n_seq: int, has_ref: bool, out: torch.Tensor, sides=()) -> torch.Tensor:
    return _run(forward_sample_steps(ctx, x, P, n_seq, has_ref, out, sides), out)


def _run(steps, out):
    for plan in steps:
        plan.launch()
    return out


def forward_sample_steps(ctx: Ctx, x: torch.Tensor, P: dict, n_seq: int, has_ref: bool, out: torch.Tensor, sides=()):
    h, w = x.shape[-2:]
    h3, w3 = h // 4, w // 4
    dev = x.device
    lanes = _lanes(ctx, sides)
    if ctx.for_stage("enc").batched_available():
        yield from forward_batch_steps(ctx, x[None], P, n_seq, [not has_ref], out[None], sides)
        return
    multi = ctx.for_stage("swin").swin_multi_available()
    with _side_lanes(lanes):
        lv = None
        if has_ref:
            with torch.cuda.stream(lanes[-1]):
                lv = reference_pyramid(ctx, x[n_seq + 1], P)
        cat = FMap(torch.empty(h3 * w3, 128 * n_seq, device=dev), h3, w3, 128 * n_seq)
        mid = x[n_seq // 2]
        e0 = enc(ctx, mid, P)
        f_mid = enc(ctx, ctx.rl_prior(mid, 5, 0.01), P, extra=e0, out=cat.view(0, 128))
        others = [i for i in range(n_seq) if i != n_seq // 2]

        def neighbour(i, out=None):
            e = enc(ctx, x[i], P)
            return enc(ctx, ctx.rl_prior(x[i], 1, 0.01), P, extra=e, out=out)

        if multi:
            fb = BMap.empty(len(others), h3, w3, 128, dev)
            for k, i in enumerate(others):
                with torch.cuda.stream(lanes[k % len(lanes)]):
                    neighbour(i, fb.map(k))
        else:
            _swin_calls(ctx, f_mid, [partial(neighbour, i) for i in others], P, cat, lanes)
    if multi:
        yield from _fuse_tail(ctx, f_mid, fb, cat, lv, P, out, lanes)
    else:
        yield from _tail(ctx, cat, lv, P, out)


def forward_batch_steps(ctx: Ctx, x: torch.Tensor, P: dict, n_seq: int, zero_ref: list, out: torch.Tensor, sides=(), max_maps: int = 16):
    B = x.shape[0]
    h, w = x.shape[-2:]
    h3, w3 = h // 4, w // 4
    dev = x.device
    lanes = _lanes(ctx, sides)
    others = [i for i in range(n_seq) if i != n_seq // 2]
    b0 = 0
    while b0 < B:
        group, maps = [], 0
        while b0 + len(group) < B:
            need = 2 + 2 * len(others) + (0 if zero_ref[b0 + len(group)] else 1)
            if group and maps + need > max_maps:
                break
            group.append(b0 + len(group))
            maps += need
        frames, first = [], {}
        for b in group:
            first[b] = len(frames)
            mid = x[b, n_seq // 2]
            frames += [mid, ctx.rl_prior(mid, 5, 0.01)]
            for i in others:
                frames += [x[b, i], ctx.rl_prior(x[b, i], 1, 0.01)]
            if not zero_ref[b]:
                frames.append(x[b, n_seq + 1])
        lv1, lv2, lv3 = enc_batched(ctx, frames, P)
        del frames
        for b in group:
            m0 = first[b]
            cat = FMap(torch.empty(h3 * w3, 128 * n_seq, device=dev), h3, w3, 128 * n_seq)
            f_mid = FMap(ctx.add(lv3.map(m0 + 1).t, lv3.map(m0).t), h3, w3, 128)
            cat.t[:, :128].copy_(f_mid.t)
            fb = BMap.empty(len(others), h3, w3, 128, dev)
            for k in range(len(others)):
                ctx.add(lv3.map(m0 + 3 + 2 * k).t, lv3.map(m0 + 2 + 2 * k).t, out=fb.map(k).t)
            mr = m0 + 2 + 2 * len(others)
            lv = None if zero_ref[b] else (lv1.map(mr), lv2.map(mr), lv3.map(mr))
            yield from _fuse_tail(ctx, f_mid, fb, cat, lv, P, out[b], lanes)
        b0 += len(group)


def _fuse_tail(ctx: Ctx, f_mid: FMap, fb: BMap, cat: FMap, lv, P: dict, out: torch.Tensor, lanes: list):
    if ctx.for_stage("swin").swin_multi_available():
        swin_multi(ctx, SwinX(ctx, f_mid, P["swin"]), fb, P["swin"], [cat.view(128 * slot, 128) for slot in range(1, fb.B + 1)])
    else:
        with _side_lanes(lanes, fork=False):
            _swin_calls(ctx, f_mid, [fb.map(k) for k in range(fb.B)], P, cat, lanes)
    yield from _tail(ctx, cat, lv, P, out)


def _tail(ctx: Ctx, cat: FMap, lv, P: dict, out: torch.Tensor):
    fw = P["fusion"]
    ff = ctx.igemm(cat, fw["w"], fw["b"], 128)
    plan = search_plan(ctx, ff, lv[2]) if lv is not None else self_plan(ctx, ff)
    yield plan
    if lv is not None:
        s, t3, t2, t1 = search_finish(ctx, plan, ff, *lv)
    else:
        s, t3, t2, t1 = self_finish(ctx, plan, ff, P)
    decode(ctx, ff, s, t3, t2, t1, P, out)


def encode_raw(ctx: Ctx, frame: torch.Tensor, P: dict) -> FMap:
    return enc(ctx, frame, P)


def encode_sum(ctx: Ctx, frame: torch.Tensor, iters: int, e_raw: FMap, P: dict) -> FMap:
    return enc(ctx, ctx.rl_prior(frame, iters, 0.01), P, extra=e_raw)


def reference_pyramid(ctx: Ctx, frame: torch.Tensor, P: dict):
    lv1 = in_block(ctx, frame, P["inBlock"])
    lv2 = enc_stage(ctx, lv1, P["encoder_first"])
    return lv1, lv2, enc_stage(ctx, lv2, P["encoder_second"])


def fuse_and_decode(ctx: Ctx, f_mid: FMap, feats: list, lv, P: dict, n_seq: int, out: torch.Tensor, sides=()) -> torch.Tensor:
    return _run(fuse_and_decode_steps(ctx, f_mid, feats, lv, P, n_seq, out, sides), out)


def fuse_and_decode_steps(ctx: Ctx, f_mid: FMap, feats: list, lv, P: dict, n_seq: int, out: torch.Tensor, sides=()):
    h3, w3 = f_mid.H, f_mid.W
    dev = f_mid.t.device
    lanes = _lanes(ctx, sides)
    cat = FMap(torch.empty(h3 * w3, 128 * n_seq, device=dev), h3, w3, 128 * n_seq)
    cat.t[:, :128].copy_(f_mid.t)
    fb = BMap(torch.cat([f.t for f in feats]), len(feats), h3, w3, 128)
    yield from _fuse_tail(ctx, f_mid, fb, cat, lv, P, out, lanes)


def forward_swint(ctx: Ctx, x: torch.Tensor, P: dict, n_seq: int, out: torch.Tensor, sides=()) -> torch.Tensor:
    h, w = x.shape[-2:]
    h3, w3 = h // 4, w // 4
    dev = x.device
    lanes = _lanes(ctx, sides if n_seq > 1 else ())
    with _side_lanes(lanes):
        cat = FMap(torch.empty(h3 * w3, 128 * n_seq, device=dev), h3, w3, 128 * n_seq)
        f_mid = enc(ctx, x[n_seq // 2], P, out=cat.view(0, 128))
        if n_seq == 1:
            f_trans = FMap.empty(h3, w3, 128, dev)
            swin(ctx, SwinX(ctx, f_mid, P["swin"]), f_mid, P["swin"], out=f_trans)
            cat = FMap(ctx.add(f_mid.t, f_trans.t), h3, w3, 128)
        else:
            _swin_calls(ctx, f_mid, [partial(enc, ctx, x[i], P) for i in range(n_seq) if i != n_seq // 2], P, cat, lanes)
    fw = P["conv"]
    ff = ctx.igemm(cat, fw["w"], fw["b"], 128)
    dctx = ctx.for_stage("decode")
    dec1 = dec_stage(dctx, dec_stage(dctx, ff, P["decoder_second"]), P["decoder_first"])
    ob = P["outBlock"]
    octx = dctx.for_stage("out")
    f = _resblocks(octx, dec1, ob["blocks"])
    return octx.for_stage("tail").conv5_out(f, ob["tail_w"], ob["tail_b"], out, ob.get("tail_w32"), ob.get("tail_b32"))
```

speinet_amd/ops.py:

```python
from __future__ import annotations

import ctypes as C
import dataclasses
from typing import Optional

import numpy as np
import torch

from . import _lib, y4m
from . import light as _light
from .pack import BF16, F16, F32, LP_DTYPE, PackedW, fmt_of

ACT_NONE, ACT_RELU, ACT_GELU = 0, 1, 2
CONV, CONV_T = 0, 1

PRECISIONS = ("f32", "bf16x3", "bf16", "f16")
CORR_PRECISIONS = ("bf16x3", "single", "top2")
_CORR_ALIASES = {"bf16": "single", "bf16r": "top2", "f16": "single"}


class FMap:
    __slots__ = ("t", "H", "W", "C", "ld", "off")

    def __init__(self, t: torch.Tensor, H: int, W: int, C_: int, off: int = 0):
        assert t.is_cuda and t.dtype in (torch.float32, torch.bfloat16, torch.float16) and t.is_contiguous() and t.dim() == 2 and t.shape[0] == H * W
        self.t, self.H, self.W, self.C, self.ld, self.off = t, H, W, C_, t.shape[1], off
        assert off + C_ <= self.ld

    @staticmethod
    def empty(H: int, W: int, C_: int, device, dtype=torch.float32) -> "FMap":
        return FMap(torch.empty(H * W, C_, device=device, dtype=dtype), H, W, C_)

    @property
    def lp(self) -> bool:
        return self.t.dtype != torch.float32

    @property
    def fmt(self) -> int:
        return fmt_of(self.t.dtype)

    def view(self, off: int, C_: int) -> "FMap":
        return FMap(self.t, self.H, self.W, C_, self.off + off)

    @property
    def ptr(self) -> int:
        return self.t.data_ptr() + self.t.element_size() * self.off

    def dense(self) -> torch.Tensor:
        return self.t[:, self.off:self.off + self.C].float().reshape(self.H, self.W, self.C)

    def nchw(self) -> torch.Tensor:
        return self.dense().permute(2, 0, 1).unsqueeze(0).contiguous()

    @staticmethod
    def from_nchw(x: torch.Tensor) -> "FMap":
        if x.dim() == 4:
            x = x[0]
        c, h, w = x.shape
        return FMap(x.permute(1, 2, 0).reshape(h * w, c).contiguous().float(), h, w, c)


class BMap:
    __slots__ = ("t", "B", "H", "W", "C")

    def __init__(self, t: torch.Tensor, B: int, H: int, W: int, C_: int):
        assert t.is_cuda and t.is_contiguous() and t.shape == (B * H * W, C_)
        self.t, self.B, self.H, self.W, self.C = t, B, H, W, C_

    @staticmethod
    def empty(B: int, H: int, W: int, C_: int, device, dtype=torch.float32) -> "BMap":
        return BMap(torch.empty(B * H * W, C_, device=device, dtype=dtype), B, H, W, C_)

    @property
    def fmt(self) -> int:
        return fmt_of(self.t.dtype)

    def map(self, b: int) -> FMap:
        n = self.H * self.W
        return FMap(self.t[b * n:(b + 1) * n], self.H, self.W, self.C)


def _vp(p) -> C.c_void_p:
    return C.c_void_p(p)


class _timed:
    def __init__(self, ctx: "Ctx", name: str):
        self.on = ctx.profile is not None and name in ctx.profile
        self.ctx, self.name = ctx, name

    def __enter__(self):
        if self.on:
            self.s = torch.cuda.Event(enable_timing=True)
            self.e = torch.cuda.Event(enable_timing=True)
            self.s.record(torch.cuda.current_stream(self.ctx.device))
        return self

    def __exit__(self, *a):
        if self.on:
            self.e.record(torch.cuda.current_stream(self.ctx.device))
            self.ctx.profile[self.name].append((self.s, self.e))
        return False


def _tensor_bytes(x) -> int:
    t = x.t if hasattr(x, "t") else x
    return t.numel() * t.element_size() if torch.is_tensor(t) else 0


def _conv_sub(method: str, a, k, out):
    if method == "conv5_in":
        return "level1", 2.0 * 25 * 3 * 32 * a[0].shape[-2] * a[0].shape[-1], _tensor_bytes(a[0]) + _tensor_bytes(out)
    if method == "conv5_out":
        return "level1", 2.0 * 25 * 32 * 3 * a[0].H * a[0].W, _tensor_bytes(a[0]) + 12 * a[0].H * a[0].W
    src, n = a[0], a[3]
    ks = a[4] if len(a) > 4 else k.get("ksize", 1)
    if n == 32 and src.C == 32 and ks == 5 and k.get("stride", a[5] if len(a) > 5 else 1) == 1:
        maps = getattr(src, "B", 1)
        return "level1", 2.0 * 25 * 32 * 32 * maps * src.H * src.W, _tensor_bytes(src) + _tensor_bytes(out)
    return "rest", 0.0, 0


def _family(name: str):
    def deco(fn):
        def wrapper(self, *a, **k):
            pr = self.profile
            if pr is None or "families" not in pr:
                return fn(self, *a, **k)
            st = torch.cuda.current_stream(self.device)
            s_, e_ = torch.cuda.Event(enable_timing=True), torch.cuda.Event(enable_timing=True)
            s_.record(st)
            out = fn(self, *a, **k)
            e_.record(st)
            pr["families"].setdefault(name, []).append((s_, e_))
            if name == "conv":
                sub, fl, by = _conv_sub(fn.__name__, a, k, out)
                rec = pr.setdefault("conv_sub", {}).setdefault(sub, {"events": [], "flops": 0.0, "bytes": 0})
                rec["events"].append((s_, e_))
                rec["flops"] += fl
                rec["bytes"] += by
            return out
        wrapper.__name__, wrapper.__doc__ = fn.__name__, fn.__doc__
        return wrapper
    return deco


def frame_metrics(u8: torch.Tensor, gt_hwc: torch.Tensor, border: int = 4) -> torch.Tensor:
    assert u8.is_cuda and u8.dtype == torch.uint8 and u8.dim() == 3 and u8.shape[2] == 3 and u8.is_contiguous()
    h, w = u8.shape[:2]
    assert gt_hwc.shape == u8.shape and gt_hwc.dtype == torch.uint8 and gt_hwc.device == u8.device and gt_hwc.is_contiguous()
    lib = _lib.lib()
    n = lib.spei_frame_metrics_ws_doubles(h, w, border)
    if n < 0:
        raise ValueError(f"frame {w}x{h} with border {border} is smaller than the 11x11 SSIM window")
    dev = u8.device
    ws = torch.empty(n, dtype=torch.float64, device=dev)
    res = torch.empty(2, dtype=torch.float64, device=dev)
    with torch.cuda.device(dev):
        st = C.c_void_p(torch.cuda.current_stream(dev).cuda_stream)
        _lib.check(lib.spei_frame_metrics(_vp(u8.data_ptr()), _vp(gt_hwc.data_ptr()), h, w, border, _vp(ws.data_ptr()), _vp(res.data_ptr()),
                                          st), "spei_frame_metrics")
    return res


def padded_size(n: int) -> int:
    return -(-n // 20) * 20


def frames_u8_in(u8: torch.Tensor, out: Optional[torch.Tensor] = None, gray: bool = False, planes: bool = True):
    assert u8.is_cuda and u8.dtype == torch.uint8 and u8.dim() in (3, 4) and (planes or gray)
    fr = u8 if u8.dim() == 4 else u8.unsqueeze(0)
    n, h, w, c = fr.shape
    assert c == 3 and fr.stride()[1:] == (w * 3, 3, 1), "frames must be packed [H,W,3] (any frame stride)"
    hp, wp = padded_size(h), padded_size(w)
    dev = u8.device
    if planes:
        if out is None:
            out = torch.empty(n, 3, hp, wp, device=dev)
        assert out.is_cuda and out.device == dev and out.dtype == torch.float32 and out.is_contiguous() and out.numel() == n * 3 * hp * wp
    else:
        out = None
    g = torch.empty(n, h, w, device=dev) if gray else None
    lib = _lib.lib()
    with torch.cuda.device(dev):
        st = C.c_void_p(torch.cuda.current_stream(dev).cuda_stream)
        _lib.check(lib.spei_frames_u8_in(_vp(fr.data_ptr()), fr.stride(0), _vp(out.data_ptr() if out is not None else 0),
                                         _vp(g.data_ptr() if g is not None else 0), n, h, w, st), "spei_frames_u8_in")
    return out, g


def frame_pair_stats(u8: torch.Tensor, prev: Optional[torch.Tensor] = None):
    assert u8.is_cuda and u8.dtype == torch.uint8 and u8.dim() == 4
    n, h, w, c = u8.shape
    assert c == 3 and u8.stride()[1:] == (w * 3, 3, 1), "frames must be packed [H,W,3] (any frame stride)"
    dev = u8.device
    assert prev is None or (prev.device == dev and prev.dtype == torch.uint8 and tuple(prev.shape) == (h, w, 3) and prev.is_contiguous())
    pairs = n if prev is not None else n - 1
    hist = torch.empty(n, 64, dtype=torch.int32, device=dev)
    sad = torch.empty(pairs, dtype=torch.int64, device=dev)
    lib = _lib.lib()
    with torch.cuda.device(dev):
        st = C.c_void_p(torch.cuda.current_stream(dev).cuda_stream)
        _lib.check(lib.spei_frame_pair_stats(_vp(u8.data_ptr()), u8.stride(0), _vp(prev.data_ptr() if prev is not None else 0), n, h, w,
                                             _vp(hist.data_ptr()), _vp(sad.data_ptr()), st), "spei_frame_pair_stats")
    return sad, hist.long()


def _depth(depth: int) -> int:
    if depth not in (10, 12):
        raise ValueError(f"depth must be 10 or 12 (bits per sample in uint16 words), got {depth!r}")
    return int(depth)


def frames_u16_in(u16: torch.Tensor, depth: int, out: Optional[torch.Tensor] = None, gray: bool = False, planes: bool = True):
    assert u16.is_cuda and u16.dtype == torch.uint16 and u16.dim() in (3, 4) and (planes or gray)
    depth = _depth(depth)
    fr = u16 if u16.dim() == 4 else u16.unsqueeze(0)
    n, h, w, c = fr.shape
    assert c == 3 and fr.stride()[1:] == (w * 3, 3, 1), "frames must be packed [H,W,3] (any frame stride)"
    hp, wp = padded_size(h), padded_size(w)
    dev = u16.device
    if planes:
        if out is None:
            out = torch.empty(n, 3, hp, wp, device=dev)
        assert out.is_cuda and out.device == dev and out.dtype == torch.float32 and out.is_contiguous() and out.numel() == n * 3 * hp * wp
    else:
        out = None
    g = torch.empty(n, h, w, device=dev) if gray else None
    lib = _lib.lib()
    with torch.cuda.device(dev):
        st = C.c_void_p(torch.cuda.current_stream(dev).cuda_stream)
        _lib.check(lib.spei_frames_u16_in(_vp(fr.data_ptr()), 2 * fr.stride(0), _vp(out.data_ptr() if out is not None else 0),
                                          _vp(g.data_ptr() if g is not None else 0), n, h, w, depth, st), "spei_frames_u16_in")
    return out, g


def frame_pair_stats_u16(u16: torch.Tensor, depth: int, prev: Optional[torch.Tensor] = None):
    assert u16.is_cuda and u16.dtype == torch.uint16 and u16.dim() == 4
    depth = _depth(depth)
    n, h, w, c = u16.shape
    assert c == 3 and u16.stride()[1:] == (w * 3, 3, 1), "frames must be packed [H,W,3] (any frame stride)"
    dev = u16.device
    assert prev is None or (prev.device == dev and prev.dtype == torch.uint16 and tuple(prev.shape) == (h, w, 3) and prev.is_contiguous())
    pairs = n if prev is not None else n - 1
    hist = torch.empty(n, 64, dtype=torch.int32, device=dev)
    sad = torch.empty(pairs, dtype=torch.int64, device=dev)
    lib = _lib.lib()
    with torch.cuda.device(dev):
        st = C.c_void_p(torch.cuda.current_stream(dev).cuda_stream)
        _lib.check(lib.spei_frame_pair_stats_u16(_vp(u16.data_ptr()), 2 * u16.stride(0), _vp(prev.data_ptr() if prev is not None else 0),
                                                 n, h, w, depth, _vp(hist.data_ptr()), _vp(sad.data_ptr()), st),
                   "spei_frame_pair_stats_u16")
    return sad, hist.long()


def window_mean_u8(u8: torch.Tensor, starts, lengths, gray: bool = False, blur: Optional[torch.Tensor] = None,
                   gt: Optional[torch.Tensor] = None, light=None):
    assert u8.is_cuda and u8.dtype == torch.uint8 and u8.dim() == 4
    t, h, w, c = u8.shape
    assert c == 3 and u8.stride()[1:] == (w * 3, 3, 1), "frames must be packed [H,W,3] (any frame stride)"
    runs_host = torch.from_numpy(np.ascontiguousarray(np.stack([np.asarray(starts), np.asarray(lengths)], axis=1).astype(np.int32)))
    m = runs_host.shape[0]
    dev = u8.device
    for name, buf in (("blur", blur), ("gt", gt)):
        assert buf is None or (buf.device == dev and buf.dtype == torch.uint8 and tuple(buf.shape) == (m, h, w, 3) and buf.is_contiguous()), name
    blur = torch.empty(m, h, w, 3, dtype=torch.uint8, device=dev) if blur is None else blur
    gt = torch.empty(m, h, w, 3, dtype=torch.uint8, device=dev) if gt is None else gt
    g = torch.empty(m, h, w, device=dev) if gray else None
    lib = _lib.lib()
    with torch.cuda.device(dev):
        runs = runs_host.to(dev)
        st = C.c_void_p(torch.cuda.current_stream(dev).cuda_stream)
        if _light.is_code(light):
            _lib.check(lib.spei_window_mean_u8(_vp(u8.data_ptr()), u8.stride(0), t, _vp(runs.data_ptr()), _vp(runs_host.data_ptr()), m,
                                               _vp(blur.data_ptr()), _vp(gt.data_ptr()), _vp(g.data_ptr() if g is not None else 0), h, w, st),
                       "spei_window_mean_u8")
        else:
            tab, tab_host = _light.device_tables(light, dev)
            _lib.check(lib.spei_window_mean_light_u8(_vp(u8.data_ptr()), u8.stride(0), t, _vp(runs.data_ptr()), _vp(runs_host.data_ptr()), m,
                                                     _vp(tab.data_ptr()), _vp(tab_host.data_ptr()), _vp(blur.data_ptr()), _vp(gt.data_ptr()),
                                                     _vp(g.data_ptr() if g is not None else 0), h, w, st), "spei_window_mean_light_u8")
    return blur, gt, g


def frame_u8_out(x: torch.Tensor, h: int, w: int, out: Optional[torch.Tensor] = None,
                 nonfinite: Optional[torch.Tensor] = None) -> torch.Tensor:
    assert x.is_cuda and x.dtype == torch.float32 and x.dim() == 3 and x.shape[0] == 3 and x.is_contiguous()
    hp, wp = x.shape[1:]
    if out is None:
        out = torch.empty(h, w, 3, dtype=torch.uint8, device=x.device)
    assert out.device == x.device and out.dtype == torch.uint8 and tuple(out.shape) == (h, w, 3) and out.is_contiguous()
    assert nonfinite is None or (nonfinite.device == x.device and nonfinite.dtype == torch.int32 and nonfinite.numel() >= 1)
    lib = _lib.lib()
    with torch.cuda.device(x.device):
        st = C.c_void_p(torch.cuda.current_stream(x.device).cuda_stream)
        _lib.check(lib.spei_frame_u8_out(_vp(x.data_ptr()), _vp(out.data_ptr()), _vp(nonfinite.data_ptr() if nonfinite is not None else 0),
                                         h, w, hp, wp, st), "spei_frame_u8_out")
    return out


def frame_u16_out(x: torch.Tensor, h: int, w: int, depth: int, out: Optional[torch.Tensor] = None,
                  nonfinite: Optional[torch.Tensor] = None) -> torch.Tensor:
    assert x.is_cuda and x.dtype == torch.float32 and x.dim() == 3 and x.shape[0] == 3 and x.is_contiguous()
    depth = _depth(depth)
    hp, wp = x.shape[1:]
    if out is None:
        out = torch.empty(h, w, 3, dtype=torch.uint16, device=x.device)
    assert out.device == x.device and out.dtype == torch.uint16 and tuple(out.shape) == (h, w, 3) and out.is_contiguous()
    assert nonfinite is None or (nonfinite.device == x.device and nonfinite.dtype == torch.int32 and nonfinite.numel() >= 1)
    lib = _lib.lib()
    with torch.cuda.device(x.device):
        st = C.c_void_p(torch.cuda.current_stream(x.device).cuda_stream)
        _lib.check(lib.spei_frame_u16_out(_vp(x.data_ptr()), _vp(out.data_ptr()), _vp(nonfinite.data_ptr() if nonfinite is not None else 0),
                                          h, w, hp, wp, depth, st), "spei_frame_u16_out")
    return out


def yuv_frame_bytes(h: int, w: int, layout: int) -> int:
    return y4m.frame_bytes(h, w, layout)


def yuv_to_rgb_u8(planar: torch.Tensor, h: int, w: int, layout: int, matrix: int, range: int,
                  out: Optional[torch.Tensor] = None) -> torch.Tensor:
    assert planar.is_cuda and planar.dtype == torch.uint8 and planar.dim() in (1, 2)
    fr = planar if planar.dim() == 2 else planar.unsqueeze(0)
    n, nb = fr.shape
    assert nb == yuv_frame_bytes(h, w, layout) and fr.stride(1) == 1, "frames must be packed planar frames (any frame stride)"
    dev = planar.device
    if out is None:
        out = torch.empty(n, h, w, 3, dtype=torch.uint8, device=dev)
    assert out.device == dev and out.dtype == torch.uint8 and tuple(out.shape) == (n, h, w, 3) and out.is_contiguous()
    lib = _lib.lib()
    with torch.cuda.device(dev):
        st = C.c_void_p(torch.cuda.current_stream(dev).cuda_stream)
        _lib.check(lib.spei_yuv_to_rgb_u8(_vp(fr.data_ptr()), fr.stride(0), _vp(out.data_ptr()), n, h, w, layout, matrix, range, st),
                   "spei_yuv_to_rgb_u8")
    return out


def rgb_u8_to_yuv(rgb: torch.Tensor, layout: int, matrix: int, range: int, out: Optional[torch.Tensor] = None) -> torch.Tensor:
    assert rgb.is_cuda and rgb.dtype == torch.uint8 and rgb.dim() == 3 and rgb.shape[2] == 3 and rgb.is_contiguous()
    h, w = rgb.shape[:2]
    nb = yuv_frame_bytes(h, w, layout)
    dev = rgb.device
    if out is None:
        out = torch.empty(nb, dtype=torch.uint8, device=dev)
    assert out.device == dev and out.dtype == torch.uint8 and tuple(out.shape) == (nb,) and out.is_contiguous()
    lib = _lib.lib()
    with torch.cuda.device(dev):
        st = C.c_void_p(torch.cuda.current_stream(dev).cuda_stream)
        _lib.check(lib.spei_rgb_u8_to_yuv(_vp(rgb.data_ptr()), _vp(out.data_ptr()), h, w, layout, matrix, range, st),
                   "spei_rgb_u8_to_yuv")
    return out


def yuv_to_rgb_u16(planar: torch.Tensor, h: int, w: int, layout: int, matrix: int, range: int, depth: int,
                   out: Optional[torch.Tensor] = None) -> torch.Tensor:
    assert planar.is_cuda and planar.dtype == torch.uint16 and planar.dim() in (1, 2)
    depth = _depth(depth)
    fr = planar if planar.dim() == 2 else planar.unsqueeze(0)
    n, ns = fr.shape
    assert ns == yuv_frame_bytes(h, w, layout) and fr.stride(1) == 1, "frames must be packed planar frames (any frame stride)"
    dev = planar.device
    if out is None:
        out = torch.empty(n, h, w, 3, dtype=torch.uint16, device=dev)
    assert out.device == dev and out.dtype == torch.uint16 and tuple(out.shape) == (n, h, w, 3) and out.is_contiguous()
    lib = _lib.lib()
    with torch.cuda.device(dev):
        st = C.c_void_p(torch.cuda.current_stream(dev).cuda_stream)
        _lib.check(lib.spei_yuv_to_rgb_u16(_vp(fr.data_ptr()), 2 * fr.stride(0), _vp(out.data_ptr()), n, h, w, layout, matrix, range, depth,
                                           st), "spei_yuv_to_rgb_u16")
    return out


def rgb_u16_to_yuv(rgb: torch.Tensor, layout: int, matrix: int, range: int, depth: int, out: Optional[torch.Tensor] = None) -> torch.Tensor:
    assert rgb.is_cuda and rgb.dtype == torch.uint16 and rgb.dim() == 3 and rgb.shape[2] == 3 and rgb.is_contiguous()
    depth = _depth(depth)
    h, w = rgb.shape[:2]
    ns = yuv_frame_bytes(h, w, layout)
    dev = rgb.device
    if out is None:
        out = torch.empty(ns, dtype=torch.uint16, device=dev)
    assert out.device == dev and out.dtype == torch.uint16 and tuple(out.shape) == (ns,) and out.is_contiguous()
    lib = _lib.lib()
    with torch.cuda.device(dev):
        st = C.c_void_p(torch.cuda.current_stream(dev).cuda_stream)
        _lib.check(lib.spei_rgb_u16_to_yuv(_vp(rgb.data_ptr()), _vp(out.data_ptr()), h, w, layout, matrix, range, depth, st),
                   "spei_rgb_u16_to_yuv")
    return out


def psnr_f32(a: torch.Tensor, b: torch.Tensor, shave: int = 4, rgb_range: float = 1.0) -> torch.Tensor:
    assert a.is_cuda and a.dtype == torch.float32 and a.dim() == 3 and a.shape[0] == 3 and a.is_contiguous()
    assert b.shape == a.shape and b.dtype == torch.float32 and b.device == a.device and b.is_contiguous()
    lib = _lib.lib()
    dev = a.device
    ws = torch.empty(PSNR_WS_DOUBLES, dtype=torch.float64, device=dev)
    res = torch.empty(2, dtype=torch.float64, device=dev)
    with torch.cuda.device(dev):
        st = C.c_void_p(torch.cuda.current_stream(dev).cuda_stream)
        _lib.check(lib.spei_psnr_f32(_vp(a.data_ptr()), _vp(b.data_ptr()), a.shape[1], a.shape[2], shave, float(rgb_range), _vp(ws.data_ptr()),
                                     _vp(res.data_ptr()), st), "spei_psnr_f32")
    return res


PSNR_WS_DOUBLES = 256


def psnr_of(sq_sum: float, count: float) -> float:
    import math
    mse = sq_sum / count
    return 100.0 if mse == 0 else 20 * math.log10(1.0 / math.sqrt(mse))


CORR_DIAG_WS_MAX = 8 << 30


class CorrPlan:
    __slots__ = ("ctx", "s", "arg", "kernel", "main", "post", "keep")

    def __init__(self, ctx, s, arg, kernel, main, post, keep):
        self.ctx, self.s, self.arg, self.kernel, self.main, self.post, self.keep = ctx, s, arg, kernel, main, post, keep

    def launch(self, profile: Optional[dict] = None) -> None:
        ctx = self.ctx if profile is None else self.ctx.replace(profile=profile)
        st = ctx._stream()
        if ctx.profile is not None:
            ctx.profile["corr_kernel"] = self.kernel
        fam = ctx.profile is not None and "families" in ctx.profile
        if fam:
            f0, f1 = torch.cuda.Event(enable_timing=True), torch.cuda.Event(enable_timing=True)
            f0.record(torch.cuda.current_stream(ctx.device))
        with _timed(ctx, "corr_argmax"):
            for fn, name, args in self.main:
                _lib.check(fn(*args, st), name)
        for fn, name, args in self.post:
            _lib.check(fn(*args, st), name)
        if fam:
            f1.record(torch.cuda.current_stream(ctx.device))
            ctx.profile["families"].setdefault("correlation", []).append((f0, f1))


@dataclasses.dataclass(frozen=True, slots=True, eq=False)
class Ctx:
    ACT_NONE, ACT_RELU, ACT_GELU = ACT_NONE, ACT_RELU, ACT_GELU
    CONV, CONV_T = CONV, CONV_T
    SPLIT_STAGES = ("glue", "dec2")

    precision: str = "f32"
    corr_precision: str = "bf16x3"
    device: Optional[torch.device] = None
    bf16_storage: bool = True
    x1_bf16: bool = True
    fuse_mlp: bool = True
    fuse_attn: bool = True
    commute_upconv: bool = True
    commute_any: bool = False
    corr_bf16: bool = True
    corr_diag: bool = True
    split_decode: bool = True
    batch_enc: bool = True
    attn_win4: bool = True
    conv32_ws: bool = True
    conv64_ws: Optional[bool] = None
    conv3_pipe: bool = True
    stage: Optional[dict] = None
    profile: Optional[dict] = None
    capture: Optional[dict] = None

    def __post_init__(self):
        put = object.__setattr__
        if self.precision not in PRECISIONS:
            raise ValueError(f"unknown precision {self.precision!r}")
        put(self, "corr_precision", _CORR_ALIASES.get(self.corr_precision, self.corr_precision))
        if self.corr_precision not in CORR_PRECISIONS:
            raise ValueError(f"unknown correlation precision {self.corr_precision!r}")
        cur = torch.cuda.current_device() if torch.cuda.is_available() else 0
        device = torch.device("cuda", cur) if self.device is None else torch.device(self.device)
        if device.type != "cuda":
            raise RuntimeError("speinet_amd runs on MI355X only (HIP kernels); there is no CPU path")
        put(self, "device", torch.device("cuda", cur) if device.index is None else device)
        for k in _BOOL_KNOBS:
            if type(getattr(self, k)) is not bool:
                put(self, k, bool(getattr(self, k)))
        if self.conv64_ws is not None:
            put(self, "conv64_ws", bool(self.conv64_ws))
        put(self, "stage", dict(self.stage) if self.stage else {})

    def replace(self, **kw) -> "Ctx":
        return dataclasses.replace(self, **kw)

    def for_stage(self, name: str) -> "Ctx":
        o = self.stage.get(name)
        if o is None and self.split_decode and self.precision == "f16" and name in self.SPLIT_STAGES:
            o = {"precision": "bf16x3", "commute_any": True}
        return self.replace(**o) if o else self

    def _tp(self, t: Optional[torch.Tensor]) -> C.c_void_p:
        if t is None:
            return C.c_void_p(0)
        assert t.is_cuda and t.is_contiguous()
        assert t.device == self.device, f"tensor on {t.device}, call context on {self.device}"
        return C.c_void_p(t.data_ptr())

    def _fp(self, f: Optional[FMap]) -> C.c_void_p:
        if f is None:
            return C.c_void_p(0)
        assert f.t.device == self.device, f"feature map on {f.t.device}, call context on {self.device}"
        return C.c_void_p(f.ptr)

    def _stream(self) -> C.c_void_p:
        assert torch.cuda.current_device() == self.device.index, \
            f"current device cuda:{torch.cuda.current_device()} != call context {self.device}"
        return C.c_void_p(torch.cuda.current_stream(self.device).cuda_stream)

    @property
    def lp16(self) -> bool:
        return self.precision in ("bf16", "f16")

    @property
    def fmt(self) -> int:
        return F16 if self.precision == "f16" else BF16

    def inter_dtype(self) -> torch.dtype:
        return LP_DTYPE[self.fmt] if (self.lp16 and self.bf16_storage) else torch.float32

    def any_nonzero(self, x: torch.Tensor, flag: torch.Tensor) -> None:
        _lib.check(_lib.lib().spei_any_nonzero(self._tp(x), x.numel(), self._tp(flag), self._stream()), "spei_any_nonzero")

    def train_batch(self, table: torch.Tensor, table_host: torch.Tensor, n_in: int, n_gt: int, input: torch.Tensor, gt: torch.Tensor,
                    patch: int, rgb_range: float = 1.0) -> None:
        nb = (n_in + n_gt) * 32
        assert table.dtype == torch.uint8 and table.numel() >= nb and not table_host.is_cuda and table_host.dtype == torch.uint8 \
            and table_host.is_contiguous() and table_host.numel() >= nb
        assert input.dtype == torch.float32 and input.numel() == n_in * 3 * patch * patch
        assert gt.dtype == torch.float32 and gt.numel() == n_gt * 3 * patch * patch
        _lib.check(_lib.lib().spei_train_batch_u8(self._tp(table), C.c_void_p(table_host.data_ptr()), n_in, n_gt, self._tp(input), self._tp(gt),
                                                  patch, float(rgb_range), self._stream()), "spei_train_batch_u8")

    def train_batch_runs(self, table: torch.Tensor, table_host: torch.Tensor, n_in: int, n_gt: int, input: torch.Tensor,
                         gt: torch.Tensor, patch: int, rgb_range: float = 1.0, light=None) -> None:
        nb = (n_in + n_gt) * 48
        assert table.dtype == torch.uint8 and table.numel() >= nb and not table_host.is_cuda and table_host.dtype == torch.uint8 \
            and table_host.is_contiguous() and table_host.numel() >= nb
        assert input.dtype == torch.float32 and input.numel() == n_in * 3 * patch * patch
        assert gt.dtype == torch.float32 and gt.numel() == n_gt * 3 * patch * patch
        if _light.is_code(light):
            _lib.check(_lib.lib().spei_train_batch_runs_u8(self._tp(table), C.c_void_p(table_host.data_ptr()), n_in, n_gt, self._tp(input),
                                                           self._tp(gt), patch, float(rgb_range), self._stream()), "spei_train_batch_runs_u8")
            return
        tab, tab_host = _light.device_tables(light, self.device)
        _lib.check(_lib.lib().spei_train_batch_runs_light_u8(self._tp(table), C.c_void_p(table_host.data_ptr()), n_in, n_gt, self._tp(tab),
                                                             C.c_void_p(tab_host.data_ptr()), self._tp(input), self._tp(gt), patch,
                                                             float(rgb_range), self._stream()), "spei_train_batch_runs_light_u8")

    def rl_prior(self, img: torch.Tensor, iters: int, lam: float = 0.01) -> torch.Tensor:
        c, h, w = img.shape
        out = torch.empty_like(img)
        scratch = torch.empty_like(img)
        _lib.check(_lib.lib().spei_rl_prior(self._tp(img), self._tp(out), self._tp(scratch), c, h, w, iters, lam, self._stream()),
                   "spei_rl_prior")
        return out

    @_family("conv")
    def conv5_in(self, img: torch.Tensor, w: torch.Tensor, b: torch.Tensor, out: Optional[FMap] = None) -> FMap:
        c, h, wd = img.shape
        assert c == 3
        if out is None:
            out = FMap.empty(h, wd, b.numel(), img.device)
        assert (out.H, out.W, out.C, out.ld, out.off) == (h, wd, b.numel(), b.numel(), 0) and not out.lp
        _lib.check(_lib.lib().spei_conv5_in(self._tp(img), self._tp(w), self._tp(b), self._fp(out), h, wd, b.numel(), self._stream()),
                   "spei_conv5_in")
        return out

    @_family("conv")
    def conv5_out(self, f: FMap, w: torch.Tensor, b: torch.Tensor, out: torch.Tensor, w32=None,
                  b32: Optional[torch.Tensor] = None) -> torch.Tensor:
        assert out.shape == (3, f.H, f.W) and out.is_contiguous() and out.dtype == torch.float32
        if self.lp16 and w32 is not None and f.C == 32:
            _lib.check(_lib.lib().spei_conv5_out_slab16(self.fmt, self._fp(f), f.ld, f.fmt, self._tp(w32.frag(self.fmt)), self._tp(b32),
                                                       self._tp(out), f.H, f.W, self._stream()), "spei_conv5_out_slab16")
            return out
        if f.lp:
            f = FMap(f.t.float(), f.H, f.W, f.C, f.off)
        _lib.check(_lib.lib().spei_conv5_out(self._fp(f), f.ld, self._tp(w), self._tp(b), self._tp(out), f.H, f.W, f.C, self._stream()),
                   "spei_conv5_out")
        return out

    def _conv3_pipe_ok(self, a, w, N: int, ksize: int, stride: int, act: int, residual, out) -> bool:
        return (self.conv3_pipe and self.lp16 and ksize == 3 and stride == 1 and N == 256 and a.C == 256 and act == ACT_NONE
                and a.H % 6 == 0 and a.W % 16 == 0 and a.H * a.W <= (1 << 21) and a.t.dtype == torch.float32 and getattr(a, "ld", 256) == 256
                and getattr(a, "off", 0) == 0 and getattr(w, "fhi", None) is not None and tuple(w.shape) == (9, 256, 256)
                and (out is None or (out.t.dtype == torch.float32 and getattr(out, "ld", 256) == 256 and getattr(out, "off", 0) == 0
                                     and out.t.data_ptr() != a.t.data_ptr()))
                and (residual is None or (residual.t.dtype == torch.float32 and getattr(residual, "ld", 256) == 256 and getattr(residual, "off", 0) == 0)))

    def _persistent_conv(self, a, w, bias, N: int, ksize: int, stride: int, act: int, residual, out, batch: int) -> bool:
        tp, lib, f = self._tp, _lib.lib(), self.fmt
        if self._conv3_pipe_ok(a, w, N, ksize, stride, act, residual, out):
            _lib.check(lib.spei_conv3x3_256_pipe16(f, tp(a.t), tp(w.frag(f)), tp(bias), tp(residual.t) if residual is not None else _vp(0),
                                                   tp(out.t), batch, a.H, a.W, self._stream()), "spei_conv3x3_256_pipe16")
            return True
        if not (ksize == 5 and stride == 1 and a.C == N and residual is None and act in (ACT_NONE, ACT_RELU) and w.fhi is not None
                and (getattr(a, "ld", N), getattr(a, "off", 0), getattr(out, "ld", N), getattr(out, "off", 0)) == (N, 0, N, 0)
                and a.t.data_ptr() != out.t.data_ptr()):
            return False
        if N == 32 and self.conv32_ws_available():
            _lib.check(lib.spei_conv32_ws16(f, tp(a.t), a.fmt, tp(w.frag(f)), tp(bias), tp(out.t), out.fmt, batch, a.H, a.W, act,
                                            self._stream()), "spei_conv32_ws16")
            return True
        if N == 64 and self.conv64_ws_available():
            _lib.check(lib.spei_conv64_ws16(f, tp(a.t), a.fmt, tp(w.frag(f)), tp(bias), tp(out.t), out.fmt, batch, a.H, a.W, act,
                                            self._stream()), "spei_conv64_ws16")
            return True
        return False

    @_family("conv")
    def igemm(self, a0: FMap, w, bias: Optional[torch.Tensor], N: int, ksize: int = 1, stride: int = 1,
              mode: int = CONV, act: int = ACT_NONE, a1: Optional[FMap] = None, residual: Optional[FMap] = None,
              rowscale: Optional[torch.Tensor] = None, out: Optional[FMap] = None, out_dtype=torch.float32,
              ln_input: bool = False) -> FMap:
        prec = self.precision
        pad = ksize // 2
        if mode == CONV:
            ho, wo = (a0.H + 2 * pad - ksize) // stride + 1, (a0.W + 2 * pad - ksize) // stride + 1
        else:
            ho, wo = a0.H * stride, a0.W * stride
        if out is None:
            out = FMap.empty(ho, wo, N, a0.t.device, out_dtype)
        assert out.H == ho and out.W == wo and out.C == N
        k0, k1 = a0.C, (a1.C if a1 is not None else 0)
        slab = prec != "f32" and mode == CONV
        assert slab or (mode == CONV_T and self.lp16) or not (a0.lp or out.lp), \
            "16-bit activations are only supported by the slab kernel"
        assert a1 is None or a1.t.dtype == a0.t.dtype
        assert residual is None or not residual.lp
        assert all(f.t.dtype in (torch.float32, LP_DTYPE[self.fmt]) for f in (a0, out)), "16-bit tensors must be in the mode's format"
        if torch.is_tensor(w):
            w = PackedW(w, a0.t.device)
        assert not ln_input or (slab and w.fhi is not None), "ln_input is a feature of the slab kernel"
        assert tuple(w.shape) == (ksize * ksize, N, k0 + k1), (tuple(w.shape), ksize, N, k0, k1)
        if a1 is not None:
            assert (a1.H, a1.W) == (a0.H, a0.W)
        if residual is not None:
            assert (residual.H, residual.W, residual.C) == (ho, wo, N)
        if rowscale is not None:
            assert rowscale.numel() == ho * wo
        tp, fp = self._tp, self._fp
        srcs = (fp(a0), a0.ld, k0, fp(a1), a1.ld if a1 is not None else 0, k1)
        lib = _lib.lib()
        if (mode == CONV and a1 is None and rowscale is None and not ln_input
                and self._persistent_conv(a0, w, bias, N, ksize, stride, act, residual, out, 1)):
            return out
        if (mode == CONV_T and self.lp16 and ksize == 3 and stride == 2 and a1 is None and residual is None
                and rowscale is None and N % 32 == 0 and k0 % 32 == 0):
            cf = w.convT_class_frags(self.fmt)
            _lib.check(lib.spei_convt2_slab16(self.fmt, fp(a0), a0.ld, k0, a0.fmt, tp(cf[(0, 0)]), tp(cf[(0, 1)]), tp(cf[(1, 0)]),
                                              tp(cf[(1, 1)]), tp(bias), fp(out), out.ld, out.fmt, a0.H, a0.W, N, act,
                                              self._stream()), "spei_convt2_slab16")
        elif (mode == CONV_T and prec == "bf16x3" and ksize == 3 and stride == 2 and a1 is None and residual is None
                and rowscale is None and N % 32 == 0 and k0 % 32 == 0 and not a0.lp and not out.lp):
            _hi, _lo, ph, pl = w.convT_class_frags_split()
            _lib.check(lib.spei_convt2_slab16x3(fp(a0), a0.ld, k0, ph, pl, tp(bias), fp(out), out.ld, a0.H, a0.W, N, act, self._stream()),
                       "spei_convt2_slab16x3")
        elif prec == "f32":
            _lib.check(lib.spei_igemm_f32(*srcs, tp(w.f32), tp(bias), fp(out), out.ld, fp(residual), residual.ld if residual is not None else 0,
                                          tp(rowscale), a0.H, a0.W, ho, wo, N, ksize, stride, pad, mode, act, self._stream()), "spei_igemm_f32")
        elif slab and w.fhi is not None:
            dims = (a0.H * a0.W, 1, ho * wo, 1) if (ksize == 1 and stride == 1) else (a0.H, a0.W, ho, wo)
            _lib.check(lib.spei_conv_slab16(
                self.fmt, *srcs, a0.fmt, tp(w.frag(self.fmt)), tp(w.flo) if prec == "bf16x3" else _vp(0), tp(bias), fp(out), out.ld,
                out.fmt, fp(residual), residual.ld if residual is not None else 0,
                tp(rowscale), *dims, N, ksize, stride, pad, act, int(ln_input), self._stream()), "spei_conv_slab16")
        else:
            raise ValueError(f"no {prec} kernel for N={N} K={k0 + k1} ksize={ksize} stride={stride} mode={mode}: N and K must be multiples "
                             "of 32; transposed convs 3x3 stride 2")
        return out

    def linear(self, x: torch.Tensor, w, b: Optional[torch.Tensor], act: int = ACT_NONE,
               residual: Optional[torch.Tensor] = None, out: Optional[torch.Tensor] = None, out_dtype=torch.float32,
               ln_input: bool = False) -> torch.Tensor:
        m, k = x.shape
        if torch.is_tensor(w):
            w = PackedW(w.reshape(1, *w.shape), x.device)
        n = w.shape[1]
        if out is None:
            out = torch.empty(m, n, device=x.device, dtype=out_dtype)
        self.igemm(FMap(x, m, 1, k), w, b, n, act=act, ln_input=ln_input,
                   residual=FMap(residual, m, 1, n) if residual is not None else None, out=FMap(out, m, 1, n))
        return out

    @_family("streaming")
    def resblock_gates(self, x1: FMap, pk: dict):
        dev = x1.t.device
        lib = _lib.lib()
        tp = self._tp
        assert x1.off == 0 and x1.ld == x1.C
        s = torch.empty(x1.C, device=dev)
        g1 = torch.empty(x1.H, x1.C, device=dev)
        g2 = torch.empty(x1.W, x1.C, device=dev)
        ws = torch.empty(lib.spei_gate_ws_floats(x1.H, x1.W, x1.C), device=dev)
        _lib.check(lib.spei_resblock_gates(self._fp(x1), x1.fmt, x1.H, x1.W, x1.C, tp(pk["se_w1"]), tp(pk["se_b1"]), tp(pk["se_w2"]),
                                           tp(pk["se_b2"]), tp(pk["cw_w"]), tp(pk["cw_bn"]), tp(pk["hc_w"]), tp(pk["hc_bn"]),
                                           tp(s), tp(g1), tp(g2), tp(ws), self._stream()), "spei_resblock_gates")
        return s, g1, g2

    def resblock(self, x: FMap, pk: dict, extra: Optional[FMap] = None, out: Optional[FMap] = None) -> FMap:
        idt = self.inter_dtype()
        c = x.C
        assert x.off == 0 and x.ld == c
        t = self.igemm(x, pk["w1"], pk["b1"], c, ksize=5, act=ACT_RELU, out_dtype=idt)
        x1 = self.igemm(t, pk["w2"], pk["b2"], c, ksize=5, out_dtype=idt if self.x1_bf16 else torch.float32)
        s, g1, g2 = self.resblock_gates(x1, pk)
        if out is None:
            out = FMap.empty(x.H, x.W, c, x.t.device)
        if extra is not None:
            assert extra.off == 0 and extra.ld == c
        self._apply(x, x1, s, g1, g2, extra, out, c)
        return out

    @_family("streaming")
    def _apply(self, x, x1, s, g1, g2, extra, out, c):
        _lib.check(_lib.lib().spei_resblock_apply(self._fp(x), self._fp(x1), x1.fmt, self._tp(s), self._tp(g1), self._tp(g2),
                                                  self._fp(extra), self._fp(out), out.ld, x.H, x.W, c, self._stream()),
                   "spei_resblock_apply")

    def batched_available(self) -> bool:
        return self.batched_kernels() and self.x1_bf16 and self.bf16_storage and self.batch_enc

    def conv32_ws_available(self) -> bool:
        return self.lp16 and self.conv32_ws

    def conv64_ws_available(self) -> bool:
        return self.lp16 and (self.conv32_ws if self.conv64_ws is None else self.conv64_ws)

    def batched_kernels(self) -> bool:
        return self.lp16

    @_family("conv")
    def igemm_batched(self, a: BMap, w, bias: torch.Tensor, N: int, ksize: int, stride: int = 1, act: int = ACT_NONE,
                      out_dtype=torch.float32, residual: Optional[BMap] = None, out: Optional[BMap] = None) -> BMap:
        assert self.batched_kernels() and not torch.is_tensor(w) and w.fhi is not None
        pad = ksize // 2
        ho, wo = (a.H + 2 * pad - ksize) // stride + 1, (a.W + 2 * pad - ksize) // stride + 1
        assert tuple(w.shape) == (ksize * ksize, N, a.C) and a.t.dtype in (torch.float32, LP_DTYPE[self.fmt])
        if out is None:
            out = BMap.empty(a.B, ho, wo, N, a.t.device, out_dtype)
        assert (out.B, out.H, out.W, out.C) == (a.B, ho, wo, N) and out.t.data_ptr() != a.t.data_ptr()
        if residual is not None:
            assert (residual.B, residual.H, residual.W, residual.C) == (a.B, ho, wo, N) and residual.t.dtype == torch.float32
            assert residual.t.data_ptr() != a.t.data_ptr()
        tp = self._tp
        if self._persistent_conv(a, w, bias, N, ksize, stride, act, residual, out, a.B):
            return out
        _lib.check(_lib.lib().spei_conv_slab16_batched(self.fmt, tp(a.t), a.C, a.fmt, tp(w.frag(self.fmt)), _vp(0), tp(bias), tp(out.t), out.fmt,
                                                       tp(residual.t) if residual is not None else _vp(0), a.B, a.H, a.W, ho, wo, N, ksize,
                                                       stride, pad, act, self._stream()),
                   "spei_conv_slab16_batched")
        return out

    def resblock_batched(self, x: BMap, pk: dict) -> BMap:
        idt = self.inter_dtype()
        c, dev = x.C, x.t.device
        lib = _lib.lib()
        tp = self._tp
        t = self.igemm_batched(x, pk["w1"], pk["b1"], c, 5, act=ACT_RELU, out_dtype=idt)
        x1 = self.igemm_batched(t, pk["w2"], pk["b2"], c, 5, out_dtype=idt)
        del t
        return self._gates_apply_batched(x, x1, pk)

    @_family("streaming")
    def _gates_apply_batched(self, x: BMap, x1: BMap, pk: dict) -> BMap:
        c, dev = x.C, x.t.device
        lib = _lib.lib()
        tp = self._tp
        s = torch.empty(x.B, c, device=dev)
        g1 = torch.empty(x.B, x.H, c, device=dev)
        g2 = torch.empty(x.B, x.W, c, device=dev)
        ws = torch.empty(x.B * lib.spei_gate_ws_floats(x.H, x.W, c), device=dev)
        _lib.check(lib.spei_resblock_gates_batched(tp(x1.t), x1.fmt, x.B, x.H, x.W, c, tp(pk["se_w1"]), tp(pk["se_b1"]), tp(pk["se_w2"]),
                                                   tp(pk["se_b2"]), tp(pk["cw_w"]), tp(pk["cw_bn"]), tp(pk["hc_w"]), tp(pk["hc_bn"]),
                                                   tp(s), tp(g1), tp(g2), tp(ws), self._stream()), "spei_resblock_gates_batched")
        out = BMap.empty(x.B, x.H, x.W, c, dev)
        _lib.check(lib.spei_resblock_apply_batched(tp(x.t), tp(x1.t), x1.fmt, tp(s), tp(g1), tp(g2), tp(out.t), x.B, x.H, x.W, c,
                                                   self._stream()), "spei_resblock_apply_batched")
        return out

    def ln_fused_available(self) -> bool:
        return self.precision != "f32"

    def attn_fused_available(self) -> bool:
        return self.lp16 and self.fuse_attn and self.bf16_storage

    def mlp_fused_available(self) -> bool:
        return self.lp16 and self.fuse_mlp

    def swin_multi_available(self) -> bool:
        return self.attn_fused_available() and self.attn_win4 and self.mlp_fused_available() and self.batched_kernels()

    @_family("swin")
    def attn_fused(self, x: torch.Tensor, yhat: torch.Tensor, bk: dict, H: int, W: int, shift: int, out: torch.Tensor) -> torch.Tensor:
        assert x.shape[0] % (H * W) == 0 and x.shape[1] == 256 and x.dtype == torch.float32 and out.shape == x.shape and out.dtype == torch.float32
        f = self.fmt
        assert yhat.shape == x.shape and yhat.dtype == LP_DTYPE[f]
        tp = self._tp
        batch = x.shape[0] // (H * W)
        if self.attn_win4:
            _lib.check(_lib.lib().spei_attn_win4_16(f, tp(x), tp(out), tp(yhat), tp(bk["wq"].frag(f)), tp(bk["bq"]), tp(bk["wkv"].frag(f)),
                                                    tp(bk["bkv"]), tp(bk["wproj"].frag(f)), tp(bk["bproj"]), tp(bk["relbias"]), batch, H, W,
                                                    shift, self._stream()), "spei_attn_win4_16")
            return out
        assert batch == 1, "the two-window kernel takes one map per launch"
        _lib.check(_lib.lib().spei_attn_fused16(f, tp(x), tp(out), tp(yhat), tp(bk["wq"].frag(f)), tp(bk["bq"]), tp(bk["wkv"].frag(f)),
                                                tp(bk["bkv"]), tp(bk["wproj"].frag(f)), tp(bk["bproj"]), tp(bk["relbias"]), H, W, shift,
                                                self._stream()), "spei_attn_fused16")
        return out

    @_family("swin")
    def mlp_fused(self, x: torch.Tensor, w1, b1: torch.Tensor, w2, b2: torch.Tensor, out: torch.Tensor) -> torch.Tensor:
        assert x.shape[1] == 256 and x.dtype == torch.float32 and out.shape == x.shape and out.dtype == torch.float32
        assert tuple(w1.shape) == (1, 512, 256) and tuple(w2.shape) == (1, 256, 512)
        tp = self._tp
        f = self.fmt
        _lib.check(_lib.lib().spei_mlp_fused16(f, tp(x), tp(out), tp(w1.frag(f)), tp(b1), tp(w2.frag(f)), tp(b2), x.shape[0], self._stream()),
                   "spei_mlp_fused16")
        return out

    def layernorm(self, x: torch.Tensor, g: Optional[torch.Tensor] = None, b: Optional[torch.Tensor] = None,
                  out: Optional[torch.Tensor] = None, out_dtype=torch.float32) -> torch.Tensor:
        assert x.shape[1] == 256 and x.is_contiguous() and x.dtype == torch.float32
        if out is None:
            out = torch.empty(x.shape, device=x.device, dtype=out_dtype)
        tp = self._tp
        _lib.check(_lib.lib().spei_layernorm256(tp(x), tp(out), fmt_of(out.dtype), tp(g), tp(b), x.shape[0], self._stream()),
                   "spei_layernorm256")
        return out

    def window_attention(self, q: torch.Tensor, kv: torch.Tensor, relbias: torch.Tensor, H: int, W: int, shift: int,
                         out: Optional[torch.Tensor] = None) -> torch.Tensor:
        assert q.shape == (H * W, 256) and kv.shape == (H * W, 512) and relbias.shape == (8, 25, 25)
        if out is None:
            out = torch.empty_like(q)
        assert q.dtype == kv.dtype == out.dtype
        tp = self._tp
        _lib.check(_lib.lib().spei_window_attention(tp(q), tp(kv), fmt_of(q.dtype), tp(relbias), tp(out), H, W, shift,
                                                    self._stream()), "spei_window_attention")
        return out

    def patch_invnorm(self, f: FMap) -> torch.Tensor:
        inv = torch.empty(f.H * f.W, device=f.t.device)
        _lib.check(_lib.lib().spei_patch_invnorm(self._fp(f), f.ld, self._tp(inv), f.H, f.W, f.C, self._stream()), "spei_patch_invnorm")
        return inv

    def corr_plan(self, lr: FMap, ref: FMap, inv_lr: torch.Tensor, inv_ref: torch.Tensor) -> "CorrPlan":
        lib = _lib.lib()
        dev = lr.t.device
        tp, fp = self._tp, self._fp
        n = lr.H * lr.W
        s = torch.empty(n, device=dev)
        arg = torch.empty(n, device=dev, dtype=torch.int32)
        dims = (lr.H, lr.W, ref.H, ref.W, lr.C)
        rescore = self.precision != "f32" and self.corr_precision == "top2" and lr.C == 128
        diag, diag_floats = False, 0
        if rescore and self.corr_diag and ref.H >= lr.H:
            diag_floats = lib.spei_corr_diag_ws_floats(lr.H, lr.W, ref.H, ref.W)
            diag = 4 * diag_floats <= min(torch.cuda.mem_get_info(dev)[0] // 4, CORR_DIAG_WS_MAX)
        ws = torch.empty(diag_floats if diag else lib.spei_corr_ws_floats(n), device=dev)
        if self.precision == "f32":
            args = (fp(lr), lr.ld, fp(ref), ref.ld, tp(inv_lr), tp(inv_ref), *dims, tp(s), tp(arg), tp(ws))
            return CorrPlan(self, s, arg, "corr_argmax_kernel (f32 MFMA)", [(lib.spei_corr_argmax, "spei_corr_argmax", args)], [],
                            (lr, ref, inv_lr, inv_ref, ws))
        split = self.corr_precision == "bf16x3"
        f16 = BF16 if (rescore and self.corr_bf16) else self.fmt
        assert f16 == BF16 or (not split and lr.C == 128), "f16 correlation: slab kernel, single / top2"
        parts = []
        for f in (lr, ref):
            hi = torch.empty(f.H * f.W, f.C, device=dev, dtype=LP_DTYPE[f16])
            lo = torch.empty_like(hi) if split else None
            _lib.check(lib.spei_split16(f16, fp(f), f.ld, tp(hi), tp(lo), f.H * f.W, f.C, self._stream()), "spei_split16")
            parts += [hi, lo]
        fname = "f16" if f16 == F16 else "bf16"
        if rescore:
            arg2 = torch.empty(n, device=dev, dtype=torch.int32)
            s2 = torch.empty(n, device=dev)
            if diag:
                main = (lib.spei_corr_diag_top2_16, "spei_corr_diag_top2_16",
                        (f16, tp(parts[0]), tp(parts[2]), tp(inv_ref), *dims, tp(s), tp(arg), tp(s2), tp(arg2), tp(ws)))
            else:
                main = (lib.spei_corr_slab_top2_16, "spei_corr_slab_top2_16",
                        (f16, tp(parts[0]), tp(parts[2]), tp(inv_lr), tp(inv_ref), *dims, tp(s), tp(arg), tp(s2), tp(arg2), tp(ws)))
            post = (lib.spei_corr_rescore, "spei_corr_rescore",
                    (fp(lr), lr.ld, fp(ref), ref.ld, tp(inv_lr), tp(inv_ref), *dims, tp(s), tp(arg), tp(s2), tp(arg2)))
            return CorrPlan(self, s, arg, f"corr_{'diag' if diag else 'slab'}_kernel<top2, {fname}>", [main], [post],
                            (lr, ref, inv_lr, inv_ref, ws, parts, s2, arg2))
        args = (tp(parts[0]), tp(parts[1]), tp(parts[2]), tp(parts[3]), tp(inv_lr), tp(inv_ref), *dims, tp(s), tp(arg), tp(ws))
        if lr.C == 128:
            main = (lib.spei_corr_slab16, "spei_corr_slab16", (f16, *args))
            kname = f"corr_slab_kernel<{'bf16x3' if split else 'top1, ' + fname}>"
        else:
            main = (lib.spei_corr_argmax_bf16, "spei_corr_argmax_bf16", args)
            kname = f"corr_bf16_kernel<{'bf16x3' if split else 'bf16'}>"
        return CorrPlan(self, s, arg, kname, [main], [], (lr, ref, inv_lr, inv_ref, ws, parts))

    def corr_argmax(self, lr: FMap, ref: FMap, inv_lr: torch.Tensor, inv_ref: torch.Tensor):
        plan = self.corr_plan(lr, ref, inv_lr, inv_ref)
        plan.launch()
        return plan.s, plan.arg

    def gather_fold(self, ref: FMap, arg: torch.Tensor, H3: int, W3: int, Hr3: int, Wr3: int, s: int) -> FMap:
        assert ref.H == Hr3 * s and ref.W == Wr3 * s
        out = FMap.empty(H3 * s, W3 * s, ref.C, ref.t.device)
        _lib.check(_lib.lib().spei_gather_fold(self._fp(ref), ref.ld, self._tp(arg), self._fp(out), out.ld, H3, W3, Hr3, Wr3, ref.C, s,
                                               self._stream()), "spei_gather_fold")
        return out

    def rot90(self, f: FMap) -> FMap:
        out = FMap.empty(f.W, f.H, f.C, f.t.device)
        _lib.check(_lib.lib().spei_rot90(self._fp(f), f.ld, self._fp(out), f.H, f.W, f.C, self._stream()), "spei_rot90")
        return out

    def upsample(self, f: FMap, s: int, act: int = ACT_NONE) -> FMap:
        out = FMap.empty(f.H * s, f.W * s, f.C, f.t.device)
        _lib.check(_lib.lib().spei_upsample_bicubic(self._fp(f), f.ld, self._fp(out), out.ld, f.H, f.W, f.C, s, act, self._stream()),
                   "spei_upsample_bicubic")
        return out

    def up_conv1x1_relu(self, f: FMap, w, b: torch.Tensor, n: int, s: int = 2) -> FMap:
        if (self.lp16 and self.commute_upconv) or self.commute_any:
            return self.upsample(self.igemm(f, w, b, n), s, act=ACT_RELU)
        return self.igemm(self.upsample(f, s), w, b, n, act=ACT_RELU)

    def add(self, a: torch.Tensor, b: torch.Tensor, out: Optional[torch.Tensor] = None) -> torch.Tensor:
        if out is None:
            out = torch.empty_like(a)
        assert out.shape == a.shape == b.shape and out.dtype == a.dtype == torch.float32
        _lib.check(_lib.lib().spei_add(self._tp(a), self._tp(b), self._tp(out), a.numel(), self._stream()), "spei_add")
        return out


_BOOL_KNOBS = tuple(f.name for f in dataclasses.fields(Ctx) if f.type in (bool, "bool"))
```

Baseline: 41.66.

## Hand off encoder outputs in 16-bit via routed resblock apply and fused epilogues

Adds a routed resblock-apply kernel that computes the final residual output for selected batch maps, optionally sums a partner map, and writes directly into fp32 concat slices and/or 16-bit buffers. This removes separate apply, add and cast passes at the encoder handoff. It also adds a double-layernorm kernel and bicubic upsample with 16-bit output so that search-branch intermediates are stored in half precision. The new path is gated by a handoff16 knob that defaults to on. The trade-off is more complex routing logic, and FMA contraction changes in the apply and layernorm arithmetic may slightly alter numerics.

```diff
diff --git a/include/speinet_hip.h b/include/speinet_hip.h
--- a/include/speinet_hip.h
+++ b/include/speinet_hip.h
@@ -102,8 +102,25 @@
 int spei_resblock_apply_batched(const float* x, const void* x1, int x1_fmt, const float* s, const float* g1, const float* g2, float* out,
                                 int batch, int H, int W, int C, spei_stream_t stream);
 
+#define SPEI_APPLY_MAX_ROUTES 16
+typedef struct {
+    float* out32;
+    void* out16;
+    int32_t ld32;
+    int32_t src;
+    int32_t partner;
+    int32_t reserved;
+} SpeiApplyRoute;
+typedef struct {
+    SpeiApplyRoute r[SPEI_APPLY_MAX_ROUTES];
+} SpeiApplyRoutes;
+int spei_resblock_apply_routed(int fmt, const float* x, const void* x1, int x1_fmt, const float* s, const float* g1, const float* g2,
+                               const SpeiApplyRoute* routes, int nroutes, int batch, int H, int W, int C, spei_stream_t stream);
+
 int spei_layernorm256(const float* x, void* y, int out_fmt, const float* gamma, const float* beta, int64_t M,
                       spei_stream_t stream);
+int spei_layernorm256_twice(const float* x, void* y, int out_fmt, const float* gamma, const float* beta, int64_t M,
+                            spei_stream_t stream);
 
 int spei_window_attention(const void* q, const void* kv, int io_fmt, const float* relbias, void* out, int H, int W,
                           int shift, spei_stream_t stream);
@@ -143,6 +160,8 @@
 
 int spei_upsample_bicubic(const float* in, int ldi, float* out, int ldo, int H, int W, int C, int s, int act,
                           spei_stream_t stream);
+int spei_upsample_bicubic_fmt(const float* in, int ldi, void* out, int ldo, int out_fmt, int H, int W, int C, int s, int act,
+                              spei_stream_t stream);
 
 int spei_add(const float* a, const float* b, float* out, int64_t n, spei_stream_t stream);
 
diff --git a/speinet_amd/csrc/resblock.hip b/speinet_amd/csrc/resblock.hip
--- a/speinet_amd/csrc/resblock.hip
+++ b/speinet_amd/csrc/resblock.hip
@@ -317,6 +317,14 @@
     }
 }
 
+__device__ __forceinline__ float apply_x3(float a, float b, float sv, float u, float v) {
+    return __fmaf_rn(b, sv, __fmaf_rn(b, u, b * v)) + a;
+}
+__device__ __forceinline__ float4 apply_x3(const float4 a, const float4 b, const float4 sv, const float4 u, const float4 v) {
+    return make_float4(apply_x3(a.x, b.x, sv.x, u.x, v.x), apply_x3(a.y, b.y, sv.y, u.y, v.y), apply_x3(a.z, b.z, sv.z, u.z, v.z),
+                       apply_x3(a.w, b.w, sv.w, u.w, v.w));
+}
+
 template <typename T>
 __global__ __launch_bounds__(256) void resblock_apply_kernel(const float* __restrict__ x, const T* __restrict__ x1,
                                                              const float* __restrict__ s, const float* __restrict__ g1,
@@ -339,16 +347,52 @@
         const float4 sv = *reinterpret_cast<const float4*>(s + c);
         const float4 u = *reinterpret_cast<const float4*>(g1 + (size_t)yy * C + c);
         const float4 v = *reinterpret_cast<const float4*>(g2 + (size_t)xx * C + c);
-        float4 o;
-        o.x = (b.x * sv.x + (b.x * u.x + b.x * v.x)) + a.x;
-        o.y = (b.y * sv.y + (b.y * u.y + b.y * v.y)) + a.y;
-        o.z = (b.z * sv.z + (b.z * u.z + b.z * v.z)) + a.z;
-        o.w = (b.w * sv.w + (b.w * u.w + b.w * v.w)) + a.w;
+        float4 o = apply_x3(a, b, sv, u, v);
         if (extra) {
             const float4 e = *reinterpret_cast<const float4*>(extra + pix * C + c);
             o.x += e.x; o.y += e.y; o.z += e.z; o.w += e.w;
         }
         *reinterpret_cast<float4*>(out + pix * ldo + c) = o;
+    }
+}
+
+template <typename T, typename LP>
+__global__ __launch_bounds__(256) void resblock_apply_routed_kernel(const float* __restrict__ x, const T* __restrict__ x1,
+                                                                    const float* __restrict__ s, const float* __restrict__ g1,
+                                                                    const float* __restrict__ g2, const SpeiApplyRoutes routes,
+                                                                    int H, int W, int C) {
+    const int cg = C / 4;
+    const int64_t total = (int64_t)H * W * cg;
+    const SpeiApplyRoute rt = routes.r[blockIdx.y];
+    const size_t m0 = (size_t)rt.src, m1 = (size_t)(rt.partner < 0 ? rt.src : rt.partner);
+    const bool pair = rt.partner >= 0;
+    const float* xa = x + m0 * H * W * C;   const float* xb = x + m1 * H * W * C;
+    const T* ya = x1 + m0 * H * W * C;      const T* yb = x1 + m1 * H * W * C;
+    const float* sa = s + m0 * C;           const float* sb = s + m1 * C;
+    const float* ua = g1 + m0 * H * C;      const float* ub = g1 + m1 * H * C;
+    const float* va = g2 + m0 * W * C;      const float* vb = g2 + m1 * W * C;
+    float* const o32 = rt.out32;
+    LP* const o16 = reinterpret_cast<LP*>(rt.out16);
+    for (int64_t i = (int64_t)blockIdx.x * 256 + threadIdx.x; i < total; i += (int64_t)gridDim.x * 256) {
+        const int c = (int)(i % cg) * 4;
+        const int64_t pix = i / cg;
+        const int xx = (int)(pix % W), yy = (int)(pix / W);
+        auto xprime = [&](const float* xp, const T* yp, const float* sp, const float* up, const float* vp) {
+            const float4 a = *reinterpret_cast<const float4*>(xp + pix * C + c);
+            const f32x4 bv = ld4<T>(yp + pix * C + c);
+            const float4 b = make_float4(bv[0], bv[1], bv[2], bv[3]);
+            const float4 sv = *reinterpret_cast<const float4*>(sp + c);
+            const float4 u = *reinterpret_cast<const float4*>(up + (size_t)yy * C + c);
+            const float4 v = *reinterpret_cast<const float4*>(vp + (size_t)xx * C + c);
+            return apply_x3(a, b, sv, u, v);
+        };
+        float4 o = xprime(xa, ya, sa, ua, va);
+        if (pair) {
+            const float4 e = xprime(xb, yb, sb, ub, vb);
+            o.x += e.x; o.y += e.y; o.z += e.z; o.w += e.w;
+        }
+        if (o32) *reinterpret_cast<float4*>(o32 + pix * rt.ld32 + c) = o;
+        if (o16) *reinterpret_cast<typename lpv<LP>::x4*>(o16 + pix * C + c) = to_lp4<LP>(f32x4{o.x, o.y, o.z, o.w});
     }
 }
 
@@ -435,3 +479,38 @@
                                            float* out, int batch, int H, int W, int C, spei_stream_t stream) {
     return resblock_apply_run(x, x1, x1_fmt, s, g1, g2, nullptr, out, C, batch, H, W, C, stream);
 }
+
+template <typename LP>
+static void apply_routed_launch(const float* x, const void* x1, bool x1_lp, const float* s, const float* g1, const float* g2,
+                                const SpeiApplyRoutes& routes, dim3 grid, int H, int W, int C, hipStream_t st) {
+    if (x1_lp) hipLaunchKernelGGL((resblock_apply_routed_kernel<LP, LP>), grid, dim3(256), 0, st, x, (const LP*)x1, s, g1, g2, routes, H, W, C);
+    else hipLaunchKernelGGL((resblock_apply_routed_kernel<float, LP>), grid, dim3(256), 0, st, x, (const float*)x1, s, g1, g2, routes, H, W, C);
+}
+
+extern "C" int spei_resblock_apply_routed(int fmt, const float* x, const void* x1, int x1_fmt, const float* s, const float* g1, const float* g2,
+                                          const SpeiApplyRoute* routes, int nroutes, int batch, int H, int W, int C, spei_stream_t stream) {
+    SPEI_REQUIRE(x && x1 && s && g1 && g2 && routes, "spei_resblock_apply_routed: null pointer");
+    SPEI_REQUIRE(fmt == SPEI_BF16 || fmt == SPEI_F16, "spei_resblock_apply_routed: fmt=%d", fmt);
+    SPEI_REQUIRE(x1_fmt == SPEI_F32 || x1_fmt == fmt, "spei_resblock_apply_routed: x1_fmt=%d with fmt=%d", x1_fmt, fmt);
+    SPEI_REQUIRE(batch >= 1 && batch <= 65535 && nroutes >= 1 && nroutes <= SPEI_APPLY_MAX_ROUTES, "spei_resblock_apply_routed: batch=%d nroutes=%d",
+                 batch, nroutes);
+    SPEI_REQUIRE(C % 4 == 0 && H > 0 && W > 0, "spei_resblock_apply_routed: bad shape");
+    SPEI_REQUIRE(((uintptr_t)x | (uintptr_t)x1 | (uintptr_t)s | (uintptr_t)g1 | (uintptr_t)g2) % 16 == 0, "spei_resblock_apply_routed: 16-byte alignment required");
+    SpeiApplyRoutes rs = {};
+    for (int i = 0; i < nroutes; ++i) {
+        const SpeiApplyRoute& r = routes[i];
+        SPEI_REQUIRE(r.src >= 0 && r.src < batch && r.partner < batch && r.partner != r.src, "spei_resblock_apply_routed: route %d: src=%d partner=%d of %d maps",
+                     i, r.src, r.partner, batch);
+        SPEI_REQUIRE(r.out32 || r.out16, "spei_resblock_apply_routed: route %d has no destination", i);
+        SPEI_REQUIRE(!r.out32 || (r.ld32 >= C && r.ld32 % 4 == 0 && (uintptr_t)r.out32 % 16 == 0), "spei_resblock_apply_routed: route %d: ld32=%d", i, r.ld32);
+        SPEI_REQUIRE(!r.out16 || (uintptr_t)r.out16 % 8 == 0, "spei_resblock_apply_routed: route %d: 16-bit destination not 8-byte aligned", i);
+        rs.r[i] = r;
+    }
+    const int64_t total = (int64_t)H * W * (C / 4);
+    const int blocks = (int)((total + 255) / 256 < 8192 ? (total + 255) / 256 : 8192);
+    const dim3 grid(blocks, nroutes);
+    if (fmt == SPEI_BF16) apply_routed_launch<__bf16>(x, x1, x1_fmt != SPEI_F32, s, g1, g2, rs, grid, H, W, C, (hipStream_t)stream);
+    else apply_routed_launch<_Float16>(x, x1, x1_fmt != SPEI_F32, s, g1, g2, rs, grid, H, W, C, (hipStream_t)stream);
+    SPEI_CHECK_LAUNCH("spei_resblock_apply_routed");
+    return 0;
+}
diff --git a/speinet_amd/csrc/stencil.hip b/speinet_amd/csrc/stencil.hip
--- a/speinet_amd/csrc/stencil.hip
+++ b/speinet_amd/csrc/stencil.hip
@@ -267,7 +267,8 @@
         else o[0] = acc[0];
     }
 }
-__global__ __launch_bounds__(256) void bicubic2x_kernel(const float* __restrict__ in, int ldi, float* __restrict__ out, int ldo,
+template <typename TO>
+__global__ __launch_bounds__(256) void bicubic2x_kernel(const float* __restrict__ in, int ldi, TO* __restrict__ out, int ldo,
                                                         int H, int W, int C, int relu) {
     const int cg = C / 4;
     const int64_t total = (int64_t)H * W * cg;
@@ -312,21 +313,35 @@
                     for (int a = 1; a < 4; ++a) r = fmaf(h[py + a][e], cy[a], r);
                     acc[e] = relu ? fmaxf(r, 0.f) : r;
                 }
-                *reinterpret_cast<f32x4*>(out + ((size_t)(2 * y + py) * (2 * W) + 2 * x + px) * ldo + c) = acc;
+                TO* o = out + ((size_t)(2 * y + py) * (2 * W) + 2 * x + px) * ldo + c;
+                if constexpr (sizeof(TO) == 4) *reinterpret_cast<f32x4*>(o) = acc;
+                else *reinterpret_cast<typename lpv<TO>::x4*>(o) = to_lp4<TO>(acc);
             }
     }
 }
 
-extern "C" int spei_upsample_bicubic(const float* in, int ldi, float* out, int ldo, int H, int W, int C, int s, int act,
-                                     spei_stream_t stream) {
-    SPEI_REQUIRE(in && out && H > 0 && W > 0 && C > 0 && (s == 2 || s == 4), "spei_upsample_bicubic: bad arguments");
+static int upsample_bicubic_run(const float* in, int ldi, void* out_, int ldo, int out_fmt, int H, int W, int C, int s, int act,
+                                spei_stream_t stream) {
+    SPEI_REQUIRE(in && out_ && H > 0 && W > 0 && C > 0 && (s == 2 || s == 4), "spei_upsample_bicubic: bad arguments");
     SPEI_REQUIRE(act == SPEI_ACT_NONE || act == SPEI_ACT_RELU, "spei_upsample_bicubic: act=%d", act);
     SPEI_REQUIRE(ldi >= C && ldo >= C, "spei_upsample_bicubic: bad row strides");
+    SPEI_REQUIRE(out_fmt == SPEI_F32 || out_fmt == SPEI_BF16 || out_fmt == SPEI_F16, "spei_upsample_bicubic_fmt: out_fmt=%d", out_fmt);
     const bool v4 = (C % 4 == 0) && (ldi % 4 == 0) && (ldo % 4 == 0);
+    if (out_fmt != SPEI_F32) {
+        SPEI_REQUIRE(v4 && s == 2 && (uintptr_t)in % 16 == 0 && (uintptr_t)out_ % 8 == 0,
+                     "spei_upsample_bicubic_fmt: a 16-bit output needs s == 2, C / ldi / ldo multiples of 4 and aligned maps");
+        const int64_t tot2 = (int64_t)H * W * (C / 4);
+        const dim3 grid((unsigned)((tot2 + 255) / 256 < 8192 ? (tot2 + 255) / 256 : 8192));
+        if (out_fmt == SPEI_BF16) hipLaunchKernelGGL(bicubic2x_kernel<__bf16>, grid, dim3(256), 0, (hipStream_t)stream, in, ldi, (__bf16*)out_, ldo, H, W, C, act == SPEI_ACT_RELU);
+        else hipLaunchKernelGGL(bicubic2x_kernel<_Float16>, grid, dim3(256), 0, (hipStream_t)stream, in, ldi, (_Float16*)out_, ldo, H, W, C, act == SPEI_ACT_RELU);
+        SPEI_CHECK_LAUNCH("spei_upsample_bicubic_fmt");
+        return 0;
+    }
+    float* out = (float*)out_;
     if (v4 && s == 2 && ((uintptr_t)in | (uintptr_t)out) % 16 == 0) {
         const int64_t tot2 = (int64_t)H * W * (C / 4);
         const int blocks2 = (int)((tot2 + 255) / 256 < 8192 ? (tot2 + 255) / 256 : 8192);
-        hipLaunchKernelGGL(bicubic2x_kernel, dim3(blocks2), dim3(256), 0, (hipStream_t)stream, in, ldi, out, ldo, H, W, C, act == SPEI_ACT_RELU);
+        hipLaunchKernelGGL(bicubic2x_kernel<float>, dim3(blocks2), dim3(256), 0, (hipStream_t)stream, in, ldi, out, ldo, H, W, C, act == SPEI_ACT_RELU);
         SPEI_CHECK_LAUNCH("spei_upsample_bicubic");
         return 0;
     }
@@ -336,6 +351,16 @@
     else    hipLaunchKernelGGL(bicubic_kernel<1>, dim3(blocks), dim3(256), 0, (hipStream_t)stream, in, ldi, out, ldo, H, W, C, s, act == SPEI_ACT_RELU);
     SPEI_CHECK_LAUNCH("spei_upsample_bicubic");
     return 0;
+}
+
+extern "C" int spei_upsample_bicubic(const float* in, int ldi, float* out, int ldo, int H, int W, int C, int s, int act,
+                                     spei_stream_t stream) {
+    return upsample_bicubic_run(in, ldi, out, ldo, SPEI_F32, H, W, C, s, act, stream);
+}
+
+extern "C" int spei_upsample_bicubic_fmt(const float* in, int ldi, void* out, int ldo, int out_fmt, int H, int W, int C, int s, int act,
+                                         spei_stream_t stream) {
+    return upsample_bicubic_run(in, ldi, out, ldo, out_fmt, H, W, C, s, act, stream);
 }
 
 __global__ __launch_bounds__(256) void rot90_kernel(const float* __restrict__ in, int ldi, float* __restrict__ out, int H, int W, int C) {
diff --git a/speinet_amd/csrc/swin.hip b/speinet_amd/csrc/swin.hip
--- a/speinet_amd/csrc/swin.hip
+++ b/speinet_amd/csrc/swin.hip
@@ -1,6 +1,31 @@
 #include "common.h"
 
 namespace {
+
+__device__ __forceinline__ float4 ln256_row(const float4 v, const float4 g, const float4 b) {
+#pragma clang fp contract(off)
+    const float mean = wave_sum((v.x + v.y) + (v.z + v.w)) * (1.0f / 256.0f);
+    const float dx = v.x - mean, dy = v.y - mean, dz = v.z - mean, dw = v.w - mean;
+    const float var_eps = __fmaf_rn(wave_sum((dx * dx + dy * dy) + (dz * dz + dw * dw)), 1.0f / 256.0f, 1e-5f);
+    const float rstd = 1.0f / sqrtf(var_eps);
+    float4 o;
+    o.x = __fmaf_rn(dx * rstd, g.x, b.x);
+    o.y = __fmaf_rn(dy * rstd, g.y, b.y);
+    o.z = __fmaf_rn(dz * rstd, g.z, b.z);
+    o.w = __fmaf_rn(dw * rstd, g.w, b.w);
+    return o;
+}
+
+template <typename TO>
+__device__ __forceinline__ void ln256_store(TO* __restrict__ y, const float4 o) {
+    if constexpr (sizeof(TO) == 4) {
+        *reinterpret_cast<float4*>(y) = o;
+    } else {
+        typename lpv<TO>::x4 h;
+        h[0] = (TO)o.x; h[1] = (TO)o.y; h[2] = (TO)o.z; h[3] = (TO)o.w;
+        *reinterpret_cast<typename lpv<TO>::x4*>(y) = h;
+    }
+}
 
 template <typename TO>
 __global__ __launch_bounds__(256) void layernorm256_kernel(const float* __restrict__ x, TO* __restrict__ y,
@@ -14,22 +39,22 @@
     if (beta) b = reinterpret_cast<const float4*>(beta)[lane];
     for (int64_t m = wave; m < M; m += nwaves) {
         const float4 v = reinterpret_cast<const float4*>(x + m * 256)[lane];
-        const float mean = wave_sum((v.x + v.y) + (v.z + v.w)) * (1.0f / 256.0f);
-        const float dx = v.x - mean, dy = v.y - mean, dz = v.z - mean, dw = v.w - mean;
-        const float var = wave_sum((dx * dx + dy * dy) + (dz * dz + dw * dw)) * (1.0f / 256.0f);
-        const float rstd = 1.0f / sqrtf(var + 1e-5f);
-        float4 o;
-        o.x = dx * rstd * g.x + b.x;
-        o.y = dy * rstd * g.y + b.y;
-        o.z = dz * rstd * g.z + b.z;
-        o.w = dw * rstd * g.w + b.w;
-        if (sizeof(TO) == 4) {
-            reinterpret_cast<float4*>(y + m * 256)[lane] = o;
-        } else {
-            typename lpv<TO>::x4 h;
-            h[0] = (TO)o.x; h[1] = (TO)o.y; h[2] = (TO)o.z; h[3] = (TO)o.w;
-            reinterpret_cast<typename lpv<TO>::x4*>(y + m * 256)[lane] = h;
-        }
+        ln256_store<TO>(y + m * 256 + 4 * lane, ln256_row(v, g, b));
+    }
+}
+
+template <typename TO>
+__global__ __launch_bounds__(256) void layernorm256_twice_kernel(const float* __restrict__ x, TO* __restrict__ y,
+                                                                 const float* __restrict__ gamma, const float* __restrict__ beta,
+                                                                 int64_t M) {
+    const int lane = threadIdx.x & 63;
+    const int64_t wave = (int64_t)blockIdx.x * 4 + (threadIdx.x >> 6);
+    const int64_t nwaves = (int64_t)gridDim.x * 4;
+    const float4 one = make_float4(1.f, 1.f, 1.f, 1.f), zero = make_float4(0.f, 0.f, 0.f, 0.f);
+    const float4 g = reinterpret_cast<const float4*>(gamma)[lane], b = reinterpret_cast<const float4*>(beta)[lane];
+    for (int64_t m = wave; m < M; m += nwaves) {
+        const float4 v = reinterpret_cast<const float4*>(x + m * 256)[lane];
+        ln256_store<TO>(y + m * 256 + 4 * lane, ln256_row(ln256_row(v, g, b), one, zero));
     }
 }
 
@@ -154,6 +179,19 @@
     return 0;
 }
 
+extern "C" int spei_layernorm256_twice(const float* x, void* y, int out_fmt, const float* gamma, const float* beta, int64_t M,
+                                       spei_stream_t stream) {
+    SPEI_REQUIRE(x && y && gamma && beta && M > 0, "spei_layernorm256_twice: bad arguments");
+    SPEI_REQUIRE(out_fmt == SPEI_F32 || out_fmt == SPEI_BF16 || out_fmt == SPEI_F16, "spei_layernorm256_twice: out_fmt=%d", out_fmt);
+    const int64_t blocks = (M + 3) / 4;
+    const dim3 grid((unsigned)(blocks < 8192 ? blocks : 8192));
+    if (out_fmt == SPEI_BF16) hipLaunchKernelGGL(layernorm256_twice_kernel<__bf16>, grid, dim3(256), 0, (hipStream_t)stream, x, (__bf16*)y, gamma, beta, M);
+    else if (out_fmt == SPEI_F16) hipLaunchKernelGGL(layernorm256_twice_kernel<_Float16>, grid, dim3(256), 0, (hipStream_t)stream, x, (_Float16*)y, gamma, beta, M);
+    else hipLaunchKernelGGL(layernorm256_twice_kernel<float>, grid, dim3(256), 0, (hipStream_t)stream, x, (float*)y, gamma, beta, M);
+    SPEI_CHECK_LAUNCH("spei_layernorm256_twice");
+    return 0;
+}
+
 static int window_attention_run(const void* q, const void* kv, int io_fmt, const float* relbias, void* out, int H, int W, int shift, int batch,
                                 spei_stream_t stream) {
     SPEI_REQUIRE(q && kv && relbias && out, "spei_window_attention: null pointer");
diff --git a/speinet_amd/engine.py b/speinet_amd/engine.py
--- a/speinet_amd/engine.py
+++ b/speinet_amd/engine.py
@@ -32,9 +32,11 @@
     return enc_stage(ctx, enc_stage(ctx, in_block(ctx, frame, P["inBlock"]), P["encoder_first"]), P["encoder_second"], extra, out)
 
 
-def enc_batched(ctx: Ctx, frames: list, P: dict):
+def enc_batched(ctx: Ctx, frames: list, P: dict, refs=None, sums=None):
     ctx = ctx.for_stage("enc")
     assert ctx.batched_available()
+    if refs is not None:
+        return _enc_batched_routed(ctx, frames, P, list(refs), list(sums))
     b, (h, w) = len(frames), frames[0].shape[-2:]
     ib = P["inBlock"]
     lv1 = BMap.empty(b, h, w, ib["head_b"].numel(), frames[0].device)
@@ -54,6 +56,33 @@
     return levels
 
 
+def _enc_batched_routed(ctx: Ctx, frames: list, P: dict, refs: list, sums: list):
+    b, (h, w) = len(frames), frames[0].shape[-2:]
+    dev, idt = frames[0].device, ctx.inter_dtype()
+    ib = P["inBlock"]
+    f = BMap.empty(b, h, w, ib["head_b"].numel(), dev)
+    for i in range(b):
+        ctx.conv5_in(frames[i], ib["head_w"], ib["head_b"], out=f.map(i))
+    levels = []
+    for name in ("inBlock", "encoder_first", "encoder_second"):
+        st = P[name]
+        if name != "inBlock":
+            f = ctx.igemm_batched(f, st["head_w"], st["head_b"], st["head_b"].numel(), 5, stride=2, act=ACT_RELU)
+        for pk in st["blocks"][:-1]:
+            f = ctx.resblock_batched(f, pk)
+        keep = {r: FMap.empty(f.H, f.W, f.C, dev) for r in refs}
+        if name != "encoder_second":
+            nxt = BMap.empty(b, f.H, f.W, f.C, dev, idt)
+            routes = [(i, None, keep.get(i), nxt.map(i)) for i in range(b)]
+        else:
+            nxt = None
+            routes = [(i, j, dest, None) for i, j, dest in sums] + [(r, None, keep[r], None) for r in refs]
+        ctx.resblock_batched(f, st["blocks"][-1], routes=routes)
+        levels.append(keep)
+        f = nxt
+    return levels
+
+
 def dec_stage(ctx: Ctx, f: FMap, pk: dict) -> FMap:
     f = _resblocks(ctx, f, pk["blocks"])
     return ctx.for_stage("convt").igemm(f, pk["tail_w"], pk["tail_b"], pk["tail_b"].numel(), ksize=3, stride=2, mode=CONV_T, act=ACT_RELU)
@@ -66,6 +95,12 @@
         self.f_mid = f_mid
         self.x_first = ctx.igemm(f_mid, sw["conv_first_w"], sw["conv_first_b"], 256, ksize=3)
         self.xt0 = ctx.layernorm(self.x_first.t, sw["pe_g"], sw["pe_b"])
+
+
+def _yhat(ctx: Ctx, y_first: torch.Tensor, sw: dict, idt) -> torch.Tensor:
+    if ctx.handoff16 and ctx.lp16:
+        return ctx.layernorm_twice(y_first, sw["pe_g"], sw["pe_b"], out_dtype=idt)
+    return ctx.layernorm(ctx.layernorm(y_first, sw["pe_g"], sw["pe_b"]), out_dtype=idt)
 
 
 def swin(ctx: Ctx, sx: SwinX, feat: FMap, sw: dict, out: FMap) -> FMap:
@@ -74,10 +109,9 @@
     m = h * w
     dev = feat.t.device
     y_first = ctx.igemm(feat, sw["conv_first_w"], sw["conv_first_b"], 256, ksize=3)
-    yt = ctx.layernorm(y_first.t, sw["pe_g"], sw["pe_b"])
     idt = ctx.inter_dtype()
-    yhat = ctx.layernorm(yt, out_dtype=idt)
-    del y_first, yt
+    yhat = _yhat(ctx, y_first.t, sw, idt)
+    del y_first
     r = sx.xt0.clone()
     bufs = [torch.empty(m, 256, device=dev), torch.empty(m, 256, device=dev)]
     xh = torch.empty(m, 256, device=dev, dtype=idt)
@@ -124,10 +158,8 @@
     m = h * w
     dev = feats.t.device
     y_first = ctx.igemm_batched(feats, sw["conv_first_w"], sw["conv_first_b"], 256, 3)
-    yt = ctx.layernorm(y_first.t, sw["pe_g"], sw["pe_b"])
-    idt = ctx.inter_dtype()
-    yhat = ctx.layernorm(yt, out_dtype=idt)
-    del y_first, yt
+    yhat = _yhat(ctx, y_first.t, sw, ctx.inter_dtype())
+    del y_first
     r = sx.xt0.repeat(B, 1)
     bufs = [torch.empty(B * m, 256, device=dev), torch.empty(B * m, 256, device=dev)]
     for layer in sw["layers"]:
@@ -200,6 +232,9 @@
     g = ctx.for_stage("glue")
     g1 = ctx.for_stage("glue1")
     c = lambda name: (P[name]["w"], P[name]["b"])
+    hd = torch.float32
+    if g1.handoff16 and g1.lp16 and (g.commute_any or (g.lp16 and g.commute_upconv)):
+        hd = g1.inter_dtype()
     h3, w3 = ff.H, ff.W
     smap = FMap(s.view(h3 * w3, 1), h3, w3, 1)
     f_lv3 = g.igemm(ff, *c("conv_lv3"), 128, a1=t3, rowscale=s, residual=ff)
@@ -213,9 +248,9 @@
     dec1 = dec_stage(ctx.for_stage("dec1"), f_lv2, P["decoder_first"])
     s4 = ctx.upsample(smap, 4).t.view(-1)
     f_lv1 = g1.igemm(dec1, *c("conv_lv1"), 32, a1=t1, rowscale=s4, residual=dec1)
-    s13 = g.up_conv1x1_relu(f_v3, *c("search13"), 32)
-    s23 = g1.igemm(ctx.upsample(f_lv2, 2), *c("search33"), 32, ksize=3, act=ACT_RELU)
-    s33 = g1.igemm(f_lv1, *c("search43"), 32, ksize=3, act=ACT_RELU)
+    s13 = g.up_conv1x1_relu(f_v3, *c("search13"), 32, out_dtype=hd)
+    s23 = g1.igemm(ctx.upsample(f_lv2, 2, out_dtype=hd), *c("search33"), 32, ksize=3, act=ACT_RELU, out_dtype=hd)
+    s33 = g1.igemm(f_lv1, *c("search43"), 32, ksize=3, act=ACT_RELU, out_dtype=hd)
     acc = g1.igemm(s13, *c("search33"), 32, ksize=3, a1=s23, act=ACT_RELU, residual=f_lv1)
     g1.igemm(s13, *c("search33"), 32, ksize=3, a1=s33, act=ACT_RELU, residual=acc, out=acc)
     g1.igemm(s23, *c("search33"), 32, ksize=3, a1=s33, act=ACT_RELU, residual=acc, out=acc)
@@ -336,6 +371,24 @@
                 frames += [x[b, i], ctx.rl_prior(x[b, i], 1, 0.01)]
             if not zero_ref[b]:
                 frames.append(x[b, n_seq + 1])
+        if ctx.for_stage("enc").handoff16:
+            cats, fbs, refs, sums = {}, {}, [], []
+            for b in group:
+                m0 = first[b]
+                cats[b] = FMap(torch.empty(h3 * w3, 128 * n_seq, device=dev), h3, w3, 128 * n_seq)
+                fbs[b] = BMap.empty(len(others), h3, w3, 128, dev)
+                sums.append((m0 + 1, m0, cats[b].view(0, 128)))
+                sums += [(m0 + 3 + 2 * k, m0 + 2 + 2 * k, fbs[b].map(k)) for k in range(len(others))]
+                if not zero_ref[b]:
+                    refs.append(m0 + 2 + 2 * len(others))
+            r1, r2, r3 = enc_batched(ctx, frames, P, refs=refs, sums=sums)
+            del frames
+            for b in group:
+                mr = first[b] + 2 + 2 * len(others)
+                lv = None if zero_ref[b] else (r1[mr], r2[mr], r3[mr])
+                yield from _fuse_tail(ctx, cats[b].view(0, 128), fbs[b], cats[b], lv, P, out[b], lanes)
+            b0 += len(group)
+            continue
         lv1, lv2, lv3 = enc_batched(ctx, frames, P)
         del frames
         for b in group:
diff --git a/speinet_amd/ops.py b/speinet_amd/ops.py
--- a/speinet_amd/ops.py
+++ b/speinet_amd/ops.py
@@ -82,6 +82,14 @@
 
 def _vp(p) -> C.c_void_p:
     return C.c_void_p(p)
+
+
+APPLY_MAX_ROUTES = 16
+
+
+class _ApplyRoute(C.Structure):
+    _fields_ = [("out32", C.c_void_p), ("out16", C.c_void_p), ("ld32", C.c_int32), ("src", C.c_int32), ("partner", C.c_int32),
+                ("reserved", C.c_int32)]
 
 
 class _timed:
@@ -464,6 +472,7 @@
     conv32_ws: bool = True
     conv64_ws: Optional[bool] = None
     conv3_pipe: bool = True
+    handoff16: bool = True
     stage: Optional[dict] = None
     profile: Optional[dict] = None
     capture: Optional[dict] = None
@@ -759,7 +768,7 @@
                    "spei_conv_slab16_batched")
         return out
 
-    def resblock_batched(self, x: BMap, pk: dict) -> BMap:
+    def resblock_batched(self, x: BMap, pk: dict, routes: Optional[list] = None) -> Optional[BMap]:
         idt = self.inter_dtype()
         c, dev = x.C, x.t.device
         lib = _lib.lib()
@@ -767,10 +776,10 @@
         t = self.igemm_batched(x, pk["w1"], pk["b1"], c, 5, act=ACT_RELU, out_dtype=idt)
         x1 = self.igemm_batched(t, pk["w2"], pk["b2"], c, 5, out_dtype=idt)
         del t
-        return self._gates_apply_batched(x, x1, pk)
+        return self._gates_apply_batched(x, x1, pk, routes)
 
     @_family("streaming")
-    def _gates_apply_batched(self, x: BMap, x1: BMap, pk: dict) -> BMap:
+    def _gates_apply_batched(self, x: BMap, x1: BMap, pk: dict, routes: Optional[list] = None) -> Optional[BMap]:
         c, dev = x.C, x.t.device
         lib = _lib.lib()
         tp = self._tp
@@ -781,6 +790,20 @@
         _lib.check(lib.spei_resblock_gates_batched(tp(x1.t), x1.fmt, x.B, x.H, x.W, c, tp(pk["se_w1"]), tp(pk["se_b1"]), tp(pk["se_w2"]),
                                                    tp(pk["se_b2"]), tp(pk["cw_w"]), tp(pk["cw_bn"]), tp(pk["hc_w"]), tp(pk["hc_bn"]),
                                                    tp(s), tp(g1), tp(g2), tp(ws), self._stream()), "spei_resblock_gates_batched")
+        if routes is not None:
+            assert self.lp16 and 1 <= len(routes) <= APPLY_MAX_ROUTES
+            arr = (_ApplyRoute * len(routes))()
+            for r, (src, partner, o32, o16) in zip(arr, routes):
+                assert 0 <= src < x.B and (partner is None or (0 <= partner < x.B and partner != src)) and (o32 is not None or o16 is not None)
+                for o, dt in ((o32, torch.float32), (o16, LP_DTYPE[self.fmt])):
+                    assert o is None or ((o.H, o.W, o.C) == (x.H, x.W, c) and o.t.dtype == dt and o.t.device == self.device)
+                assert o16 is None or (o16.ld, o16.off) == (c, 0)
+                r.src, r.partner = src, -1 if partner is None else partner
+                r.out32, r.ld32 = (o32.ptr, o32.ld) if o32 is not None else (None, 0)
+                r.out16 = o16.ptr if o16 is not None else None
+            _lib.check(lib.spei_resblock_apply_routed(self.fmt, tp(x.t), tp(x1.t), x1.fmt, tp(s), tp(g1), tp(g2), arr, len(routes), x.B,
+                                                      x.H, x.W, c, self._stream()), "spei_resblock_apply_routed")
+            return None
         out = BMap.empty(x.B, x.H, x.W, c, dev)
         _lib.check(lib.spei_resblock_apply_batched(tp(x.t), tp(x1.t), x1.fmt, tp(s), tp(g1), tp(g2), tp(out.t), x.B, x.H, x.W, c,
                                                    self._stream()), "spei_resblock_apply_batched")
@@ -834,6 +857,14 @@
         tp = self._tp
         _lib.check(_lib.lib().spei_layernorm256(tp(x), tp(out), fmt_of(out.dtype), tp(g), tp(b), x.shape[0], self._stream()),
                    "spei_layernorm256")
+        return out
+
+    def layernorm_twice(self, x: torch.Tensor, g: torch.Tensor, b: torch.Tensor, out_dtype=torch.float32) -> torch.Tensor:
+        assert x.shape[1] == 256 and x.is_contiguous() and x.dtype == torch.float32 and g.numel() == b.numel() == 256
+        out = torch.empty(x.shape, device=x.device, dtype=out_dtype)
+        tp = self._tp
+        _lib.check(_lib.lib().spei_layernorm256_twice(tp(x), tp(out), fmt_of(out.dtype), tp(g), tp(b), x.shape[0], self._stream()),
+                   "spei_layernorm256_twice")
         return out
 
     def window_attention(self, q: torch.Tensor, kv: torch.Tensor, relbias: torch.Tensor, H: int, W: int, shift: int,
@@ -919,16 +950,20 @@
         _lib.check(_lib.lib().spei_rot90(self._fp(f), f.ld, self._fp(out), f.H, f.W, f.C, self._stream()), "spei_rot90")
         return out
 
-    def upsample(self, f: FMap, s: int, act: int = ACT_NONE) -> FMap:
-        out = FMap.empty(f.H * s, f.W * s, f.C, f.t.device)
-        _lib.check(_lib.lib().spei_upsample_bicubic(self._fp(f), f.ld, self._fp(out), out.ld, f.H, f.W, f.C, s, act, self._stream()),
-                   "spei_upsample_bicubic")
-        return out
-
-    def up_conv1x1_relu(self, f: FMap, w, b: torch.Tensor, n: int, s: int = 2) -> FMap:
+    def upsample(self, f: FMap, s: int, act: int = ACT_NONE, out_dtype=torch.float32) -> FMap:
+        out = FMap.empty(f.H * s, f.W * s, f.C, f.t.device, out_dtype)
+        if out_dtype == torch.float32:
+            _lib.check(_lib.lib().spei_upsample_bicubic(self._fp(f), f.ld, self._fp(out), out.ld, f.H, f.W, f.C, s, act, self._stream()),
+                       "spei_upsample_bicubic")
+        else:
+            _lib.check(_lib.lib().spei_upsample_bicubic_fmt(self._fp(f), f.ld, self._fp(out), out.ld, out.fmt, f.H, f.W, f.C, s, act,
+                                                            self._stream()), "spei_upsample_bicubic_fmt")
+        return out
+
+    def up_conv1x1_relu(self, f: FMap, w, b: torch.Tensor, n: int, s: int = 2, out_dtype=torch.float32) -> FMap:
         if (self.lp16 and self.commute_upconv) or self.commute_any:
-            return self.upsample(self.igemm(f, w, b, n), s, act=ACT_RELU)
-        return self.igemm(self.upsample(f, s), w, b, n, act=ACT_RELU)
+            return self.upsample(self.igemm(f, w, b, n), s, act=ACT_RELU, out_dtype=out_dtype)
+        return self.igemm(self.upsample(f, s), w, b, n, act=ACT_RELU, out_dtype=out_dtype)
 
     def add(self, a: torch.Tensor, b: torch.Tensor, out: Optional[torch.Tensor] = None) -> torch.Tensor:
         if out is None:
```

Result: faster. 42.26 (median of 6 runs) (+1.4%).
